# Yusheng-Xu/VGS-SVGS-Segmentation

Hardware: AMD Instinct MI355X
Metric: segmented points/sec (end-to-end VGS) (higher is better)
Workload: dtype f32

## Files before the change

### vgs-svgs-segmentation_amd/csrc/brick_table.hpp

```cpp
#ifndef BRICK_TABLE_HPP_
#define BRICK_TABLE_HPP_

#include "vgs_context.hpp"

struct Brick { unsigned long long key; unsigned long long occ; unsigned long long used; uint32_t first; uint32_t pad; };

__device__ __forceinline__ uint32_t hash_slot(uint64_t key, uint32_t hbits) {
  const uint32_t bx = (uint32_t)key & 0x1fffffu, by = (uint32_t)(key >> 21) & 0x1fffffu, bz = (uint32_t)(key >> 42);
  uint32_t h = bx * 0x9E3779B1u + by * 0x85EBCA77u + bz * 0xC2B2AE3Du;
  h ^= h >> 15;
  return (h * 0x2C1B3C6Du) >> (32 - hbits);
}

__device__ __forceinline__ unsigned long long brick_key(uint32_t nx, uint32_t ny, uint32_t nz) {
  return (((unsigned long long)(nz >> 2) << 42) | ((unsigned long long)(ny >> 2) << 21) | (unsigned long long)(nx >> 2)) + 1ull;
}
__device__ __forceinline__ int brick_local(uint32_t nx, uint32_t ny, uint32_t nz) {
  return (int)((nz & 1u) | ((ny & 1u) << 1) | ((nx & 1u) << 2) | ((nz & 2u) << 2) | ((ny & 2u) << 3) | ((nx & 2u) << 4));
}

static __global__ void k_brick_insert(const uint64_t* __restrict__ vox_code, const NodeRec* __restrict__ node, int64_t V,
                               Brick* __restrict__ table, uint32_t hbits) {
  const int64_t v = (int64_t)blockIdx.x * blockDim.x + threadIdx.x;
  const int lane = threadIdx.x & 63;
  unsigned long long key = 0ull, occ = 0ull, usd = 0ull;
  uint32_t first = 0xffffffffu;
  if (v < V) {
    const uint64_t code = vox_code[v];
    key = brick_key(vm_compact21(code >> 2), vm_compact21(code >> 1), vm_compact21(code));
    occ = 1ull << (code & 63ull);
    if (node && (node[v].flags & VGS_F_EIG)) usd = occ;
    first = (uint32_t)v;
  }
  for (int o = 1; o < 64; o <<= 1) {
    const unsigned long long ko = __shfl_up(key, o, 64), oo = __shfl_up(occ, o, 64), uo = __shfl_up(usd, o, 64);
    const uint32_t fo = (uint32_t)__shfl_up((int)first, o, 64);
    if (lane >= o && ko == key) { occ |= oo; usd |= uo; first = fo < first ? fo : first; }
  }
  const unsigned long long knext = __shfl_down(key, 1, 64);
  if (key == 0ull || (lane < 63 && knext == key)) return;
  const uint32_t mask = (1u << hbits) - 1u;
  uint32_t s = hash_slot(key, hbits);
  while (true) {
    const unsigned long long prev = atomicCAS(&table[s].key, 0ull, key);
    if (prev == 0ull || prev == key) break;
    s = (s + 1) & mask;
  }
  atomicOr(&table[s].occ, occ);
  if (usd) atomicOr(&table[s].used, usd);
  atomicMin(&table[s].first, first);
}

__device__ __forceinline__ int brick_find(const Brick* __restrict__ table, uint32_t hbits, uint32_t nx, uint32_t ny, uint32_t nz, bool* is_used) {
  const unsigned long long key = brick_key(nx, ny, nz);
  const uint32_t mask = (1u << hbits) - 1u;
  uint32_t s = hash_slot(key, hbits);
  while (true) {
    const unsigned long long k = table[s].key;
    if (k == key) break;
    if (k == 0ull) return -1;
    s = (s + 1) & mask;
  }
  const unsigned long long occ = table[s].occ;
  const int local = brick_local(nx, ny, nz);
  if (!((occ >> local) & 1ull)) return -1;
  *is_used = ((table[s].used >> local) & 1ull) != 0;
  const unsigned long long above = (local == 63) ? 0ull : (occ >> (local + 1));
  return (int)(table[s].first + (uint32_t)__popcll(above));
}


static __global__ void k_brick_clear(Brick* __restrict__ table, size_t H) {
  const size_t e = (size_t)blockIdx.x * blockDim.x + threadIdx.x;
  if (e >= H) return;
  ulonglong2* p = (ulonglong2*)&table[e];
  p[0] = make_ulonglong2(0ull, 0ull);
  p[1] = make_ulonglong2(0ull, 0x00000000ffffffffull);
}

static inline vgs_status vgs_build_bricks(vgs_ctx* c, const NodeRec* node) {
  const int64_t V = c->V;
  uint32_t hbits = 4;
  while ((1ull << hbits) < (uint64_t)(V + 16)) ++hbits;
  c->hbits = hbits;
  const size_t H = (size_t)1 << hbits;
  VGS_HIP_TRY(c, c->hkey.ensure(H * (sizeof(Brick) / 8)));
  hipLaunchKernelGGL(k_brick_clear, dim3((unsigned)((H + 255) / 256)), dim3(256), 0, c->stream, (Brick*)c->hkey.p, H);
  hipLaunchKernelGGL(k_brick_insert, dim3((unsigned)((V + 255) / 256)), dim3(256), 0, c->stream, c->vox_code.p, node, V, (Brick*)c->hkey.p, hbits);
  return VGS_OK;
}

#endif
```

### vgs-svgs-segmentation_amd/csrc/capi.hip

```cpp
#include <algorithm>
#include <cstdio>
#include <cstdlib>
#include <cstring>
#include <fstream>
#include <string>
#include <vector>

#include <dlfcn.h>

#include "vgs_context.hpp"

static thread_local std::string g_create_err;

static const char* const VGS_STAGE_NAMES[VGS_T_COUNT] = {"vgs:voxelize", "vgs:features", "vgs:adjacency", "vgs:localcut", "vgs:merge", "vgs:labels",
                                                         "vgs:total", "vgs:localcut_kernel", "vgs:supervoxels", "vgs:localcut_bulk", "", ""};
struct RoctxApi {
  int (*push)(const char*) = nullptr;
  int (*pop)() = nullptr;
  RoctxApi() {
    for (const char* name : {"librocprofiler-sdk-roctx.so.1", "librocprofiler-sdk-roctx.so", "libroctx64.so.4", "libroctx64.so"}) {
      void* h = dlopen(name, RTLD_LAZY | RTLD_LOCAL);
      if (!h) continue;
      push = (int (*)(const char*))dlsym(h, "roctxRangePushA");
      pop = (int (*)())dlsym(h, "roctxRangePop");
      if (push && pop) return;
      push = nullptr; pop = nullptr;
    }
  }
};
static const RoctxApi& roctx_api() { static const RoctxApi api; return api; }
struct RoctxRange {
  bool on;
  explicit RoctxRange(const char* name) : on(roctx_api().push != nullptr) { if (on) roctx_api().push(name); }
  ~RoctxRange() { if (on) roctx_api().pop(); }
};

template <typename F>
static vgs_status timed(vgs_ctx* c, int slot, F&& f, bool wait = true) {
  RoctxRange range(VGS_STAGE_NAMES[slot]);
  VGS_HIP_TRY(c, hipSetDevice(c->device));
  VGS_HIP_TRY(c, hipEventRecord(c->tev[slot][0], c->stream));
  c->tev_pending[slot] = false;
  vgs_status s = f();
  if (s != VGS_OK) return s;
  VGS_HIP_TRY(c, hipEventRecord(c->tev[slot][1], c->stream));
  c->tev_pending[slot] = true;
  if (wait) VGS_HIP_TRY(c, hipEventSynchronize(c->tev[slot][1]));
  return VGS_OK;
}

static vgs_status vgs_resolve_times(vgs_ctx* c) {
  for (int slot = 0; slot < VGS_T_COUNT; ++slot) {
    if (!c->tev_pending[slot]) continue;
    c->tev_pending[slot] = false;
    VGS_HIP_TRY(c, hipEventSynchronize(c->tev[slot][1]));
    float ms = 0.f;
    VGS_HIP_TRY(c, hipEventElapsedTime(&ms, c->tev[slot][0], c->tev[slot][1]));
    c->times[slot] = ms;
  }
  return VGS_OK;
}

void vgs_read_env_knobs(vgs_ctx* c) {
  VgsKnobs& k = c->K;
  auto geti = [](const char* n, int d) { const char* v = getenv(n); return v ? atoi(v) : d; };
  auto getf = [](const char* n, float d) { const char* v = getenv(n); return v ? (float)atof(v) : d; };
  auto has = [](const char* n) { return getenv(n) != nullptr; };
  k.a1_max = geti("VGS_A1MAX", k.a1_max); k.shell0 = getf("VGS_SHELL0", k.shell0); k.cap_frac = getf("VGS_CAPFRAC", k.cap_frac);
  k.dbg_stop = geti("VGS_DBG_STOP", k.dbg_stop); k.max_rounds = geti("VGS_ROUNDS", k.max_rounds); k.dbg_max_m = geti("VGS_DBG_MAXM", k.dbg_max_m); k.dbg_xl_from = geti("VGS_DBG_XL_FROM", k.dbg_xl_from);
  k.near_min_own = geti("VGS_NEARMINOWN", k.near_min_own); k.fv_blocks = geti("VGS_FV_BLOCKS", k.fv_blocks); k.only_class = geti("VGS_ONLY_CLASS", k.only_class);
  k.no_dense = has("VGS_NO_DENSE"); k.no_overlap = has("VGS_NO_OVERLAP"); k.no_near = has("VGS_NO_NEAR"); k.no_adjmasks = has("VGS_NO_ADJMASKS"); k.no_connbits = has("VGS_NO_CONNBITS"); k.no_pg_xl = has("VGS_NO_PG_XL"); k.no_sort32 = has("VGS_NO_SORT32"); k.no_pairlists = has("VGS_NO_PAIRLISTS"); k.no_vote = has("VGS_NO_VOTE"); k.vote_force = geti("VGS_VOTE_FORCE", 0); k.cross_lds_kb = geti("VGS_CROSS_LDS", k.cross_lds_kb); { int vp = geti("VGS_VOTE_PERIOD", k.vote_period); if (vp >= 2 && vp <= 4096 && (vp & (vp - 1)) == 0) k.vote_period = vp; } k.pg_wide = geti("VGS_PG_WIDE", k.pg_wide); k.pg_wide_frac = geti("VGS_PG_WIDEFRAC", k.pg_wide_frac); k.pg_min_frac = geti("VGS_PG_MINFRAC", k.pg_min_frac); k.ho_grid = geti("VGS_HO_GRID", k.ho_grid);
  k.debug = has("VGS_DEBUG");
}

static void vgs_charge_localcut_tail(vgs_ctx* c) {
  (void)vgs_resolve_times(c);
  const double t = (double)c->lc_tail.tail_ms;
  if (t > 0.0 && t < c->times[VGS_T_MERGE]) { c->times[VGS_T_LOCALCUT] += t; c->times[VGS_T_MERGE] -= t; }
  c->lc_tail.tail_ms = 0.f;
}

extern "C" {

vgs_status vgs_params_default_vgs(vgs_params* p) {
  if (!p) return VGS_E_ARG;
  std::memset(p, 0, sizeof(*p));
  p->method = 2;
  p->voxel_size = 0.15f; p->graph_size = 0.5f;
  p->sig_p = p->sig_n = p->sig_o = p->sig_e = p->sig_c = 0.2f;
  p->sig_w = 2.0f; p->cut_thred = 0.3f;
  p->points_min = 10; p->adjacency_min = 3; p->voxels_min = 3;
  p->seed_size = 0.25f; p->color_impt = 0.0f; p->spatial_impt = 0.25f; p->normal_impt = 0.75f;
  p->q7_count_as_index = 1;
  p->device = 0;
  return VGS_OK;
}

vgs_status vgs_params_default_svgs(vgs_params* p) {
  vgs_status s = vgs_params_default_vgs(p);
  if (s != VGS_OK) return s;
  p->method = 3;
  p->voxel_size = 0.05f; p->seed_size = 0.25f; p->graph_size = 0.5f;
  p->sig_w = 1.0f; p->cut_thred = 0.5f;
  p->vccs_mode = 1;
  return VGS_OK;
}

vgs_status vgs_parse_task_file(const char* path, vgs_params* p, char* in_name, char* out_name, int name_cap) {
  if (!path || !p) return VGS_E_ARG;
  std::ifstream f(path);
  if (!f.is_open()) return VGS_E_IO;
  std::vector<std::string> v;
  std::string line;
  while (std::getline(f, line)) {
    while (!line.empty() && (line.back() == '\r' || line.back() == '\n')) line.pop_back();
    v.push_back(line);
  }
  auto num = [&](size_t k) -> double { return k < v.size() ? std::atof(v[k].c_str()) : 0.0; };
  auto inum = [&](size_t k) -> int { return k < v.size() ? std::atoi(v[k].c_str()) : 0; };
  if (v.size() < 51) return VGS_E_IO;
  const int method = inum(24);
  if (method == 3) {
    if (v.size() < 61) return VGS_E_IO;
    vgs_params_default_svgs(p);
    p->voxel_size = (float)num(28); p->seed_size = (float)num(30); p->graph_size = (float)num(32);
    p->sig_p = (float)num(34); p->sig_n = (float)num(36); p->sig_o = (float)num(38); p->sig_e = (float)num(40);
    p->sig_c = (float)num(42); p->sig_w = (float)num(44);
    p->color_impt = (float)num(46); p->spatial_impt = (float)num(48); p->normal_impt = (float)num(50);
    p->cut_thred = (float)num(52);
    p->points_min = (int)num(54); p->voxels_min = inum(58); p->adjacency_min = inum(60);
  } else {
    vgs_params_default_vgs(p);
    p->voxel_size = (float)num(28); p->graph_size = (float)num(30);
    p->sig_p = (float)num(32); p->sig_n = (float)num(34); p->sig_o = (float)num(36); p->sig_e = (float)num(38);
    p->sig_c = (float)num(40); p->sig_w = (float)num(42); p->cut_thred = (float)num(44);
    p->points_min = inum(46); p->adjacency_min = inum(48); p->voxels_min = inum(50);
    p->method = 2;
  }
  if (in_name && name_cap > 0) { std::strncpy(in_name, v[15].c_str(), name_cap - 1); in_name[name_cap - 1] = 0; }
  if (out_name && name_cap > 0) { std::strncpy(out_name, v[21].c_str(), name_cap - 1); out_name[name_cap - 1] = 0; }
  return VGS_OK;
}

vgs_status vgs_create(const vgs_params* p, vgs_ctx** out) {
  if (!p || !out) return VGS_E_ARG;
  *out = nullptr;
  if (!(p->voxel_size > 0.f) || !(p->graph_size > 0.f) || !(p->sig_w != 0.f) || (p->method != 2 && p->method != 3)) {
    g_create_err = "vgs_create: voxel_size, graph_size must be > 0, sig_w != 0, method 2 or 3";
    return VGS_E_ARG;
  }
  if (p->vccs_mode != 0 && p->vccs_mode != 1) { g_create_err = "vgs_create: vccs_mode must be 0 (synchronous variant) or 1 (PCL's order)"; return VGS_E_ARG; }
  int ndev = 0;
  hipError_t e = hipGetDeviceCount(&ndev);
  if (e != hipSuccess || ndev <= 0) {
    g_create_err = std::string("vgs_create: no HIP device (") + hipGetErrorString(e) + "); this engine has no CPU path";
    return VGS_E_HIP;
  }
  if (p->device < 0 || p->device >= ndev) { g_create_err = "vgs_create: bad device ordinal"; return VGS_E_ARG; }
  vgs_ctx* c = new (std::nothrow) vgs_ctx();
  if (!c) return VGS_E_NOMEM;
  c->P = *p;
  c->device = p->device;
  int prio_lo = 0, prio_hi = 0;
  if (hipSetDevice(c->device) != hipSuccess || hipStreamCreateWithFlags(&c->stream, hipStreamNonBlocking) != hipSuccess ||
      hipDeviceGetStreamPriorityRange(&prio_lo, &prio_hi) != hipSuccess ||
      hipStreamCreateWithPriority(&c->stream2, hipStreamNonBlocking, prio_hi) != hipSuccess ||
      hipStreamCreateWithPriority(&c->stream3, hipStreamNonBlocking, prio_hi) != hipSuccess ||
      hipStreamCreateWithPriority(&c->stream4, hipStreamNonBlocking, prio_hi) != hipSuccess) {
    g_create_err = "vgs_create: hipSetDevice/hipStreamCreate failed";
    vgs_destroy(c);
    return VGS_E_HIP;
  }
  if (hipHostMalloc(&c->pin, 4096, hipHostMallocDefault) != hipSuccess) c->pin = nullptr;
  bool ok = hipStreamCreateWithFlags(&c->s_h2d, hipStreamNonBlocking) == hipSuccess &&
            hipStreamCreateWithFlags(&c->s_d2h, hipStreamNonBlocking) == hipSuccess &&
            hipEventCreateWithFlags(&c->ev_h2d, hipEventDisableTiming) == hipSuccess &&
            hipEventCreateWithFlags(&c->ev_d2h, hipEventDisableTiming) == hipSuccess &&
            hipEventCreateWithFlags(&c->ev_rb, hipEventDisableTiming) == hipSuccess &&
            hipEventCreateWithFlags(&c->ev_ho, hipEventDisableTiming) == hipSuccess &&
            hipEventCreateWithFlags(&c->ev_ho2, hipEventDisableTiming) == hipSuccess &&
            hipEventCreateWithFlags(&c->ev_fork, hipEventDisableTiming) == hipSuccess &&
            hipEventCreateWithFlags(&c->ev_join, hipEventDisableTiming) == hipSuccess;
  for (int i = 0; ok && i < 16; ++i) ok = hipEventCreate(&c->ev[i]) == hipSuccess;
  for (int i = 0; ok && i < VGS_T_COUNT; ++i) ok = hipEventCreate(&c->tev[i][0]) == hipSuccess && hipEventCreate(&c->tev[i][1]) == hipSuccess;
  if (!ok) { g_create_err = "vgs_create: hipStreamCreate/hipEventCreate failed"; vgs_destroy(c); return VGS_E_HIP; }
  vgs_read_env_knobs(c);
  *out = c;
  return VGS_OK;
}

void vgs_destroy(vgs_ctx* c) {
  if (!c) return;
  (void)hipSetDevice(c->device);
  if (c->stream) (void)hipStreamSynchronize(c->stream);
  if (c->stream2) (void)hipStreamSynchronize(c->stream2);
  if (c->stream3) (void)hipStreamSynchronize(c->stream3);
  if (c->stream4) (void)hipStreamSynchronize(c->stream4);
  if (c->s_h2d) (void)hipStreamSynchronize(c->s_h2d);
  if (c->s_d2h) (void)hipStreamSynchronize(c->s_d2h);
  c->xyz_buf[0].release(); c->xyz_buf[1].release(); c->pt_label_alt.release(); c->grow_state.release();
  c->code_a.release(); c->code_b.release(); c->perm_a.release(); c->perm_b.release(); c->sort_tmp.release();
  c->head_flag.release(); c->pt_vox.release(); c->vox_tile.release(); c->vox_code.release(); c->vox_start.release();
  c->xs.release(); c->ys.release(); c->zs.release();
  c->node.release(); c->used_ids.release(); c->used_rank.release();
  c->hkey.release(); c->hval.release(); c->offsets.release(); c->adj_masks.release(); c->adj_gtab.release(); c->adj_nvals.release(); c->adj_nrank.release(); c->adj_key.release(); c->adj_off.release(); c->adj_cnt.release(); c->adj_mused.release();
  c->nl_cnt.release(); c->nl_tot.release(); c->nl_ent.release(); c->lc_ctab.release(); c->pl_state.release(); c->pl_ent.release(); c->pl_work.release();
  c->sd_key.release(); c->sd_ids.release(); c->sd_vp.release(); c->sd_seg.release(); c->sd_tmp.release(); c->sd_part.release();
  c->sd_npts.release(); c->sd_nnodes.release(); c->sd_bbox.release(); c->sd_eig8.release(); c->sd_cen.release(); c->sd_cov.release(); c->sd_eval.release(); c->sd_evec.release();
  c->sd_apos.release(); c->sd_mom.release();
  c->sf_in.release(); c->sf_min.release(); c->sf_max.release(); c->sf_cls.release(); c->sf_maj.release(); c->sf_part.release(); c->sf_anchor.release(); c->sf_idx.release();
  c->sf_mean.release(); c->sf_var.release(); c->sf_nvalid.release(); c->sf_hist.release();
  c->sb_part.release(); c->sbt_in.release(); c->sbt_frame.release(); c->sbt_out.release(); c->sbt_idx.release();
  for (int f = 0; f < 2; ++f) { c->sb_frame[f].release(); c->sb_lo[f].release(); c->sb_hi[f].release(); c->sb_half[f].release(); c->sb_center[f].release(); }
  c->sg_lab.release(); c->sg_nrec.release(); c->sg_ridx.release(); c->sg_ework.release(); c->sg_meta.release(); c->sg_roff.release(); c->sg_rkey.release(); c->sg_rec.release(); c->sg_part.release(); c->sg_tmp.release();
  c->sg_ab.release(); c->sg_nodes.release(); c->sg_npairs.release(); c->sg_nfin.release(); c->sg_wsum.release(); c->sg_wmin.release(); c->sg_wmax.release();
  c->cmp_ref.release(); c->cmp_cell_i32.release(); c->cmp_ref_i32.release(); c->cmp_seg_i32.release(); c->cmp_cell_n.release(); c->cmp_ref_i64.release(); c->cmp_seg_i64.release();
  c->cmp_ref_iou.release(); c->cmp_seg_iou.release(); c->cmp_key.release(); c->cmp_meta.release(); c->cmp_work.release(); c->cmp_cstart.release(); c->cmp_rowstart.release();
  c->cmp_rsort.release(); c->cmp_rstart.release(); c->cmp_tmp.release();
  c->rf_label.release(); c->rf_batches.release(); c->rf_start.release(); c->rf_ids.release(); c->rf_cnt.release(); c->rf_nall.release();
  c->rf_rows.release(); c->rf_counts.release();
  c->ps_in.release(); c->ps_nnodes.release(); c->ps_key.release(); c->ps_val.release(); c->ps_seg.release(); c->ps_nn.release(); c->ps_tmp.release();
  c->ps_meta.release(); c->ps_part.release(); c->ps_d.release(); c->ps_f.release(); c->ps_npts.release();
  c->cl_off.release(); c->cl_idx.release(); c->conn.release(); c->evals.release(); c->lc_pending.release(); c->lc_defer.release(); c->lc_defer_flag.release(); c->csize.release(); c->attach.release(); c->cc_flags.release(); c->parent.release(); c->csz.release();
  c->vc_cen.release(); c->vc_nrm.release(); c->vc_dist.release(); c->vc_state.release(); c->vc_tile_start.release(); c->vc_cell.release(); c->vc_plive.release(); c->vc_tile_of.release(); c->vc_tchg.release(); c->vc_nbr_tiles.release(); c->vc_halo.release(); c->vc_tile_meta.release(); c->vc_pool.release(); c->vc_ring.release(); c->vc_dbg.release(); c->vc_label.release();
  c->vc_seedkey.release(); c->vc_sums.release(); c->vc_count.release(); c->vc_accu.release(); c->vc_alive.release();
  c->sv_label.release(); c->sv_key_a.release(); c->sv_key_b.release(); c->cell_code_a.release(); c->cell_code_b.release();
  c->cell_id_a.release(); c->cell_id_b.release(); c->cell_start.release();
  c->owned.release(); c->straddle.release(); c->mixsrc.release(); c->bnd_code.release(); c->bnd_root.release(); c->root_label.release();
  c->bnd_code2.release(); c->bnd_root2.release(); c->bnd_cnt.release(); c->broot.release();
  c->kept_rank.release(); c->vox_label.release(); c->pt_label.release(); c->counters.release(); c->work_ids.release();
  if (c->pin) (void)hipHostFree(c->pin);
  for (int i = 0; i < 16; ++i) if (c->ev[i]) (void)hipEventDestroy(c->ev[i]);
  for (int i = 0; i < VGS_T_COUNT; ++i) for (int k = 0; k < 2; ++k) if (c->tev[i][k]) (void)hipEventDestroy(c->tev[i][k]);
  if (c->stream) (void)hipStreamDestroy(c->stream);
  if (c->stream2) (void)hipStreamDestroy(c->stream2);
  if (c->stream3) (void)hipStreamDestroy(c->stream3);
  if (c->stream4) (void)hipStreamDestroy(c->stream4);
  if (c->s_h2d) (void)hipStreamDestroy(c->s_h2d);
  if (c->s_d2h) (void)hipStreamDestroy(c->s_d2h);
  if (c->ev_h2d) (void)hipEventDestroy(c->ev_h2d);
  if (c->ev_rb) (void)hipEventDestroy(c->ev_rb);
  if (c->ev_ho) (void)hipEventDestroy(c->ev_ho);
  if (c->ev_ho2) (void)hipEventDestroy(c->ev_ho2);
  if (c->ev_fork) (void)hipEventDestroy(c->ev_fork);
  if (c->ev_join) (void)hipEventDestroy(c->ev_join);
  if (c->ev_d2h) (void)hipEventDestroy(c->ev_d2h);
  delete c;
}

vgs_status vgs_set_params(vgs_ctx* c, const vgs_params* p) {
  if (!c || !p) return VGS_E_ARG;
  if (!(p->voxel_size > 0.f) || !(p->graph_size > 0.f) || !(p->sig_w != 0.f)) { c->err = "vgs_set_params: voxel_size, graph_size > 0, sig_w != 0"; return VGS_E_ARG; }
  if (p->method != c->P.method || p->device != c->P.device) { c->err = "vgs_set_params: method and device are fixed at vgs_create"; return VGS_E_ARG; }
  if (p->vccs_mode != 0 && p->vccs_mode != 1) { c->err = "vgs_set_params: vccs_mode must be 0 (synchronous variant) or 1 (PCL's order)"; return VGS_E_ARG; }
  int keep = ST_SEGMENTED;
  const vgs_params& o = c->P;
  if (p->cut_thred != o.cut_thred || p->sig_p != o.sig_p || p->sig_n != o.sig_n || p->sig_o != o.sig_o || p->sig_e != o.sig_e ||
      p->sig_c != o.sig_c || p->sig_w != o.sig_w || p->adjacency_min != o.adjacency_min || p->voxels_min != o.voxels_min ||
      p->q7_count_as_index != o.q7_count_as_index)
    keep = ST_ADJACENCY;
  if (p->graph_size != o.graph_size) keep = ST_FEATURES;
  if (p->points_min != o.points_min) keep = ST_VOXELS;
  if (p->voxel_size != o.voxel_size || p->seed_size != o.seed_size || p->color_impt != o.color_impt ||
      p->spatial_impt != o.spatial_impt || p->normal_impt != o.normal_impt || p->vccs_mode != o.vccs_mode)
    keep = ST_POINTS;
  if (c->stage > keep) c->stage = keep;
  if (keep < ST_SEGMENTED) { c->sd_valid = false; c->sb_valid[0] = c->sb_valid[1] = false; c->sg_valid = false; c->cmp_valid = false; c->rf_valid = false; c->cmp_own_cells = -1; c->sg_halo_valid = false; c->sg_own_K = -1; c->rf_halo_valid = false; c->rf_band_n = -1; }
  if (keep == ST_POINTS && c->P.method == 3 && !c->sv_labels_external) { c->sv_have_labels = false; c->sv_max_label = 0; c->sv_label_n = -1; }
  c->P = *p;
  return VGS_OK;
}

const char* vgs_last_error_string(const vgs_ctx* c) { return c ? c->err.c_str() : g_create_err.c_str(); }

static vgs_status set_points_common(vgs_ctx* c, int64_t n, int32_t stride_bytes) {
  if (n < 0 || (stride_bytes != 12 && stride_bytes != 16)) { c->err = "set_points: n >= 0 and stride_bytes 12 or 16 required"; return VGS_E_ARG; }
  if (n >= (int64_t)1 << 31) { c->err = "set_points: more than 2^31-1 points"; return VGS_E_UNSUPPORTED; }
  c->N = n;
  c->stride_f = stride_bytes / 4;
  c->stage = ST_POINTS;
  c->sd_valid = false;
  c->sb_valid[0] = c->sb_valid[1] = false;
  c->sg_valid = false; c->cmp_valid = false; c->rf_valid = false; c->cmp_own_cells = -1; c->sg_halo_valid = false; c->sg_own_K = -1; c->rf_halo_valid = false; c->rf_band_n = -1;
  c->grid_covers = false;
  c->counts[VGS_N_POINTS] = n;
  for (int i = 0; i < VGS_T_COUNT; ++i) { c->times[i] = 0; c->tev_pending[i] = false; }
  c->sv_have_labels = false; c->sv_labels_external = false; c->sv_max_label = 0; c->sv_label_n = -1;
  c->n_own = -1; c->own_first = 0;
  return VGS_OK;
}

vgs_status vgs_set_points(vgs_ctx* c, const float* xyz_host, int64_t n, int32_t stride_bytes) {
  if (!c || (!xyz_host && n > 0)) return VGS_E_ARG;
  VGS_HIP_TRY(c, hipSetDevice(c->device));
  vgs_status s = set_points_common(c, n, stride_bytes);
  if (s != VGS_OK) return s;
  DevBuf<float>& buf = c->xyz_buf[c->xyz_cur];
  VGS_HIP_TRY(c, buf.ensure((size_t)n * c->stride_f + 4));
  if (n > 0) VGS_HIP_TRY(c, hipMemcpyAsync(buf.p, xyz_host, (size_t)n * stride_bytes, hipMemcpyHostToDevice, c->stream));
  VGS_HIP_TRY(c, hipStreamSynchronize(c->stream));
  c->xyz = buf.p;
  return VGS_OK;
}

vgs_status vgs_stage_points(vgs_ctx* c, const float* xyz_host, int64_t n, int32_t stride_bytes) {
  if (!c || (!xyz_host && n > 0)) return VGS_E_ARG;
  if (n < 0 || (stride_bytes != 12 && stride_bytes != 16)) { c->err = "vgs_stage_points: n >= 0 and stride_bytes 12 or 16 required"; return VGS_E_ARG; }
  if (n >= (int64_t)1 << 31) { c->err = "vgs_stage_points: more than 2^31-1 points"; return VGS_E_UNSUPPORTED; }
  VGS_HIP_TRY(c, hipSetDevice(c->device));
  if (c->staged) VGS_HIP_TRY(c, hipEventSynchronize(c->ev_h2d));
  DevBuf<float>& buf = c->xyz_buf[1 - c->xyz_cur];
  VGS_HIP_TRY(c, buf.ensure((size_t)n * (stride_bytes / 4) + 4));
  if (n > 0) VGS_HIP_TRY(c, hipMemcpyAsync(buf.p, xyz_host, (size_t)n * stride_bytes, hipMemcpyHostToDevice, c->s_h2d));
  VGS_HIP_TRY(c, hipEventRecord(c->ev_h2d, c->s_h2d));
  c->staged = true; c->staged_n = n; c->staged_stride = stride_bytes;
  return VGS_OK;
}

vgs_status vgs_commit_points(vgs_ctx* c) {
  if (!c) return VGS_E_ARG;
  if (!c->staged) { c->err = "vgs_commit_points: no staged cloud (vgs_stage_points first)"; return VGS_E_STATE; }
  VGS_HIP_TRY(c, hipSetDevice(c->device));
  VGS_HIP_TRY(c, hipStreamWaitEvent(c->stream, c->ev_h2d, 0));
  vgs_status s = set_points_common(c, c->staged_n, c->staged_stride);
  if (s != VGS_OK) return s;
  c->xyz_cur = 1 - c->xyz_cur;
  c->xyz = c->xyz_buf[c->xyz_cur].p;
  c->staged = false;
  return VGS_OK;
}

vgs_status vgs_host_alloc(void** p, uint64_t bytes) {
  if (!p) return VGS_E_ARG;
  *p = nullptr;
  return hipHostMalloc(p, bytes > 0 ? (size_t)bytes : 1, hipHostMallocDefault) == hipSuccess ? VGS_OK : VGS_E_NOMEM;
}
vgs_status vgs_host_free(void* p) { return (!p || hipHostFree(p) == hipSuccess) ? VGS_OK : VGS_E_HIP; }
vgs_status vgs_host_register(void* p, uint64_t bytes) {
  if (!p || bytes == 0) return VGS_E_ARG;
  return hipHostRegister(p, (size_t)bytes, hipHostRegisterDefault) == hipSuccess ? VGS_OK : VGS_E_HIP;
}
vgs_status vgs_host_unregister(void* p) { return (p && hipHostUnregister(p) == hipSuccess) ? VGS_OK : VGS_E_HIP; }

vgs_status vgs_set_points_device(vgs_ctx* c, const float* xyz_dev, int64_t n, int32_t stride_bytes) {
  if (!c || (!xyz_dev && n > 0)) return VGS_E_ARG;
  VGS_HIP_TRY(c, hipSetDevice(c->device));
  vgs_status s = set_points_common(c, n, stride_bytes);
  if (s != VGS_OK) return s;
  c->xyz = xyz_dev;
  return VGS_OK;
}

}

static vgs_status do_voxelize(vgs_ctx* c, bool wait) {
  if (!c) return VGS_E_ARG;
  if (c->stage < ST_POINTS) { c->err = "vgs_voxelize: no input cloud (setInputCloud/getCloudPointNum first)"; return VGS_E_STATE; }
  vgs_status s = timed(c, VGS_T_VOXELIZE, [&] { return vgs_stage_voxelize(c); }, wait);
  if (s == VGS_OK) c->stage = ST_VOXELS;
  return s;
// ... 111 lines not shown
    for (uint32_t x : cnt) e += x;
    c->counts[VGS_N_ADJ] = e;
  }
  if (c->stage >= ST_SEGMENTED && c->U > 0 && c->counts[VGS_N_PAIRS] < 0) {
    std::vector<uint32_t> ev((size_t)c->U);
    VGS_HIP_TRY(c, hipMemcpy(ev.data(), c->evals.p, ev.size() * 4, hipMemcpyDeviceToHost));
    int64_t tot = 0;
    for (uint32_t x : ev) tot += x;
    c->counts[VGS_N_PAIRS] = tot;
  }
  for (int i = 0; i < VGS_N_COUNTS; ++i) counts[i] = c->counts[i];
  return VGS_OK;
}

vgs_status vgs_get_stage_times(vgs_ctx* c, double* ms) {
  if (!c || !ms) return VGS_E_ARG;
  { vgs_status sr = vgs_resolve_times(c); if (sr != VGS_OK) return sr; }
  if (c->P.method == 2 && c->stage >= ST_SEGMENTED)
    c->times[VGS_T_TOTAL] = c->times[VGS_T_VOXELIZE] + c->times[VGS_T_FEATURES] + c->times[VGS_T_ADJACENCY] + c->times[VGS_T_LOCALCUT] + c->times[VGS_T_MERGE];
  for (int i = 0; i < VGS_T_COUNT; ++i) ms[i] = c->times[i];
  return VGS_OK;
}

vgs_status vgs_get_schedule_counters(vgs_ctx* c, int64_t* out) { return vgs_get_schedule_counters_ex(c, out, 8); }

vgs_status vgs_get_schedule_counters_ex(vgs_ctx* c, int64_t* out, int32_t n) {
  if (!c || !out || n < 0 || n > 16) return VGS_E_ARG;
  for (int i = 0; i < n; ++i) out[i] = c->lc_diag[i];
  return VGS_OK;
}

vgs_status vgs_get_bbox(vgs_ctx* c, double* b) {
  if (!c || !b) return VGS_E_ARG;
  if (c->stage < ST_VOXELS) { c->err = "vgs_get_bbox: voxelize first"; return VGS_E_STATE; }
  for (int a = 0; a < 3; ++a) { b[a] = c->box.min[a]; b[3 + a] = c->box.max[a]; }
  return VGS_OK;
}

vgs_status vgs_get_voxel_table(vgs_ctx* c, uint32_t* key, int32_t* start, int32_t* point_idx) {
  if (!c) return VGS_E_ARG;
  if (c->stage < ST_VOXELS) { c->err = "vgs_get_voxel_table: voxelize first"; return VGS_E_STATE; }
  VGS_HIP_TRY(c, hipSetDevice(c->device));
  if (key && c->V > 0) {
    std::vector<uint64_t> code((size_t)c->V);
    VGS_HIP_TRY(c, hipMemcpy(code.data(), c->vox_code.p, code.size() * 8, hipMemcpyDeviceToHost));
    for (int64_t v = 0; v < c->V; ++v) {
      key[3 * v + 0] = vm_compact21(code[v] >> 2);
      key[3 * v + 1] = vm_compact21(code[v] >> 1);
      key[3 * v + 2] = vm_compact21(code[v]);
    }
  }
  if (start) {
    if (c->V > 0) VGS_HIP_TRY(c, hipMemcpy(start, c->vox_start.p, (size_t)(c->V + 1) * 4, hipMemcpyDeviceToHost));
    else start[0] = 0;
  }
  if (point_idx && c->Nf > 0) VGS_HIP_TRY(c, hipMemcpy(point_idx, c->perm_b.p, (size_t)c->Nf * 4, hipMemcpyDeviceToHost));
  return VGS_OK;
}

vgs_status vgs_get_voxel_centers(vgs_ctx* c, float* center) {
  if (!c || !center) return VGS_E_ARG;
  if (c->stage < ST_VOXELS) { c->err = "vgs_get_voxel_centers: voxelize first"; return VGS_E_STATE; }
  if (c->V == 0) return VGS_OK;
  std::vector<uint64_t> code((size_t)c->V);
  VGS_HIP_TRY(c, hipMemcpy(code.data(), c->vox_code.p, code.size() * 8, hipMemcpyDeviceToHost));
  const float res_f = c->P.voxel_size;
  const float mn[3] = {(float)c->box.min[0], (float)c->box.min[1], (float)c->box.min[2]};
  for (int64_t v = 0; v < c->V; ++v) {
    center[3 * v + 0] = vm_voxel_center(vm_compact21(code[v] >> 2), res_f, mn[0]);
    center[3 * v + 1] = vm_voxel_center(vm_compact21(code[v] >> 1), res_f, mn[1]);
    center[3 * v + 2] = vm_voxel_center(vm_compact21(code[v]), res_f, mn[2]);
  }
  return VGS_OK;
}

vgs_status vgs_get_point_voxel(vgs_ctx* c, int32_t* out) {
  if (!c || !out) return VGS_E_ARG;
  if (c->stage < ST_VOXELS) { c->err = "vgs_get_point_voxel: voxelize first"; return VGS_E_STATE; }
  if (c->N == 0) return VGS_OK;
  if (c->Nf == 0) {
    for (int64_t j = 0; j < c->N; ++j) out[j] = -1;
    return VGS_OK;
  }
  std::vector<uint32_t> perm((size_t)c->N), pv((size_t)c->N);
  VGS_HIP_TRY(c, hipMemcpy(perm.data(), c->perm_b.p, perm.size() * 4, hipMemcpyDeviceToHost));
  VGS_HIP_TRY(c, hipMemcpy(pv.data(), c->pt_vox.p, pv.size() * 4, hipMemcpyDeviceToHost));
  for (int64_t j = 0; j < c->N; ++j) out[perm[j]] = (pv[j] == 0xffffffffu) ? -1 : (int32_t)pv[j];
  return VGS_OK;
}

vgs_status vgs_get_attributes(vgs_ctx* c, float* centroid, float* normal, float* eigen8, uint8_t* used) {
  if (!c) return VGS_E_ARG;
  if (c->stage < ST_FEATURES) { c->err = "vgs_get_attributes: features first"; return VGS_E_STATE; }
  if (c->V == 0) return VGS_OK;
  std::vector<NodeRec> nd((size_t)c->V);
  VGS_HIP_TRY(c, hipMemcpy(nd.data(), c->node.p, nd.size() * sizeof(NodeRec), hipMemcpyDeviceToHost));
  for (int64_t v = 0; v < c->V; ++v) {
    for (int a = 0; a < 3; ++a) {
      if (centroid) centroid[3 * v + a] = nd[v].c[a];
      if (normal) normal[3 * v + a] = nd[v].n[a];
    }
    if (eigen8) for (int a = 0; a < 8; ++a) eigen8[8 * v + a] = nd[v].f[a];
    if (used) used[v] = (nd[v].flags & VGS_F_EIG) ? 1 : 0;
  }
  return VGS_OK;
}

}

static vgs_status vgs_build_lists(vgs_ctx* c, int32_t which, std::vector<std::vector<int32_t>>& L, bool ordered = false) {
  const int64_t V = c->V, U = c->U;
  if (which == 0 && c->P.method == 2 && V > 0) {
    VGS_HIP_TRY(c, hipSetDevice(c->device));
    L.assign((size_t)V, {});
    const int64_t chunk = std::min<int64_t>(V, 65536);
    DevBuf<uint64_t> fk; DevBuf<uint32_t> fc, fn, fid;
    VGS_HIP_TRY(c, fk.ensure((size_t)chunk * c->adj_stride)); VGS_HIP_TRY(c, fc.ensure(chunk)); VGS_HIP_TRY(c, fn.ensure(chunk)); VGS_HIP_TRY(c, fid.ensure(chunk));
    std::vector<uint32_t> ids((size_t)chunk), cnt((size_t)chunk);
    std::vector<uint64_t> keys((size_t)chunk * c->adj_stride);
    vgs_status st = VGS_OK;
    for (int64_t v0 = 0; v0 < V && st == VGS_OK; v0 += chunk) {
      const int64_t m = std::min(chunk, V - v0);
      for (int64_t k = 0; k < m; ++k) ids[(size_t)k] = (uint32_t)(v0 + k);
      if (hipMemcpy(fid.p, ids.data(), (size_t)m * 4, hipMemcpyHostToDevice) != hipSuccess) { st = VGS_E_HIP; break; }
      st = vgs_run_adjacency(c, true, fk.p, fc.p, fn.p, c->adj_r2, fid.p, m);
      if (st == VGS_OK && hipStreamSynchronize(c->stream) != hipSuccess) st = VGS_E_HIP;
      if (st == VGS_OK && (hipMemcpy(cnt.data(), fc.p, (size_t)m * 4, hipMemcpyDeviceToHost) != hipSuccess ||
                           hipMemcpy(keys.data(), fk.p, (size_t)m * c->adj_stride * 8, hipMemcpyDeviceToHost) != hipSuccess)) st = VGS_E_HIP;
      if (st != VGS_OK) break;
      for (int64_t k = 0; k < m; ++k) {
        std::vector<int32_t>& l = L[(size_t)(v0 + k)];
        l.resize(cnt[(size_t)k]);
        for (uint32_t q = 0; q < cnt[(size_t)k]; ++q) l[q] = (int32_t)(uint32_t)keys[(size_t)k * c->adj_stride + q];
      }
    }
    fk.release(); fc.release(); fn.release(); fid.release();
    if (st == VGS_E_HIP) c->err = "vgs_get_lists: full adjacency pass failed";
    return st;
  }
  std::vector<uint32_t> used_ids((size_t)U), cnt((size_t)U);
  std::vector<uint64_t> keys;
  std::vector<uint8_t> flag;
  std::vector<int32_t> attach;
  if (ordered && which >= 1 && U > 0) {
    VGS_HIP_TRY(c, hipSetDevice(c->device));
    VGS_HIP_TRY(c, hipMemcpy(used_ids.data(), c->used_ids.p, (size_t)U * 4, hipMemcpyDeviceToHost));
    std::vector<uint16_t> ord;
    std::vector<uint32_t> kk, lcnt;
    std::vector<int32_t> lids;
    const uint8_t* lflag = which == 1 ? (const uint8_t*)nullptr : c->conn.p + (size_t)U * c->adj_stride;
    vgs_status so = vgs_cut_order(c, ord, kk, true, lflag, &lcnt, &lids);
    if (so != VGS_OK) return so;
    L.assign((size_t)V, {});
    size_t at = 0;
    for (int64_t u = 0; u < U; ++u) {
      L[used_ids[(size_t)u]].assign(lids.begin() + (ptrdiff_t)at, lids.begin() + (ptrdiff_t)(at + lcnt[(size_t)u]));
      at += lcnt[(size_t)u];
    }
    if (which == 3) {
      attach.resize((size_t)V);
      VGS_HIP_TRY(c, hipMemcpy(attach.data(), c->attach.p, (size_t)V * 4, hipMemcpyDeviceToHost));
      for (int64_t i = 0; i < V; ++i)
        if (attach[i] >= 0) { L[i].push_back(attach[i]); L[attach[i]].push_back((int32_t)i); }
    }
    return VGS_OK;
  }
  if (U > 0) {
    VGS_HIP_TRY(c, hipSetDevice(c->device));
    VGS_HIP_TRY(c, hipMemcpy(used_ids.data(), c->used_ids.p, (size_t)U * 4, hipMemcpyDeviceToHost));
    keys.resize((size_t)U * c->adj_stride);
// ... 176 lines not shown
```

### vgs-svgs-segmentation_amd/csrc/clusters.hip

```cpp
#include <cstring>
#include <string.h>

#include <rocprim/rocprim.hpp>

#include "vgs_context.hpp"

__global__ void k_cluster_keys(const uint32_t* __restrict__ pt_vox, const int32_t* __restrict__ vox_label, int64_t nf, uint32_t K,
                               uint32_t* __restrict__ key) {
  const int64_t j = (int64_t)blockIdx.x * blockDim.x + threadIdx.x;
  if (j >= nf) return;
  const uint32_t v = pt_vox[j];
  const int32_t l = v == 0xffffffffu ? -1 : vox_label[v];
  key[j] = l < 0 ? K : (uint32_t)l;
}
__global__ void k_cluster_offsets(const uint32_t* __restrict__ key, int64_t nf, uint32_t K, int64_t* __restrict__ off) {
  const uint32_t k = blockIdx.x * blockDim.x + threadIdx.x;
  if (k > K) return;
  int64_t lo = 0, hi = nf;
  while (lo < hi) { const int64_t mid = (lo + hi) >> 1; if (key[mid] < k) lo = mid + 1; else hi = mid; }
  off[k] = lo;
}

vgs_status vgs_clusters_on_device(vgs_ctx* c) {
  if (c->cl_valid) return VGS_OK;
  const int64_t K = c->counts[VGS_N_KEPT], nf = c->Nf;
  VGS_HIP_TRY(c, hipSetDevice(c->device));
  VGS_HIP_TRY(c, c->cl_off.ensure((size_t)K + 2));
  VGS_HIP_TRY(c, c->cl_idx.ensure((size_t)(nf > 0 ? nf : 1)));
  if (nf == 0 || K == 0) {
    VGS_HIP_TRY(c, hipMemsetAsync(c->cl_off.p, 0, ((size_t)K + 1) * sizeof(int64_t), c->stream));
    VGS_HIP_TRY(c, hipStreamSynchronize(c->stream));
    c->cl_valid = true;
    return VGS_OK;
  }
  VGS_HIP_TRY(c, c->code_a.ensure((size_t)nf)); VGS_HIP_TRY(c, c->code_b.ensure((size_t)nf));
  uint32_t* key_in = (uint32_t*)c->code_a.p;
  uint32_t* key_out = key_in + nf;
  uint32_t* val_out = (uint32_t*)c->cl_idx.p;
  const int TB = 256;
  const unsigned nb = (unsigned)((nf + TB - 1) / TB);
  hipLaunchKernelGGL(k_cluster_keys, dim3(nb), dim3(TB), 0, c->stream, c->pt_vox.p, c->vox_label.p, nf, (uint32_t)K, key_in);
  unsigned bits = 1;
  while (bits < 32 && (1ull << bits) <= (unsigned long long)K) ++bits;
  size_t tmp = 0;
  VGS_HIP_TRY(c, rocprim::radix_sort_pairs(nullptr, tmp, key_in, key_out, c->perm_b.p, val_out, (size_t)nf, 0, bits, c->stream));
  VGS_HIP_TRY(c, c->sort_tmp.ensure(tmp));
  VGS_HIP_TRY(c, rocprim::radix_sort_pairs(c->sort_tmp.p, tmp, key_in, key_out, c->perm_b.p, val_out, (size_t)nf, 0, bits, c->stream));
  hipLaunchKernelGGL(k_cluster_offsets, dim3((unsigned)((K + 1 + TB - 1) / TB)), dim3(TB), 0, c->stream, key_out, nf, (uint32_t)K, c->cl_off.p);
  VGS_HIP_TRY(c, hipGetLastError());
  VGS_HIP_TRY(c, hipStreamSynchronize(c->stream));
  c->cl_valid = true;
  return VGS_OK;
}

extern "C" vgs_status vgs_get_clusters_device(vgs_ctx* c, const int64_t** offsets_dev, const int32_t** point_idx_dev) {
  if (!c || !offsets_dev || !point_idx_dev) return VGS_E_ARG;
  if (c->stage < ST_SEGMENTED) { c->err = "vgs_get_clusters_device: segment first (drawColorMapofPointsinClusters precedes getClusterIdx, VS:1006)"; return VGS_E_STATE; }
  vgs_status s = vgs_clusters_on_device(c);
  if (s != VGS_OK) return s;
  *offsets_dev = c->cl_off.p;
  *point_idx_dev = c->cl_idx.p;
  return VGS_OK;
}
```

### vgs-svgs-segmentation_amd/csrc/localcut.hip

```cpp
#include <algorithm>
#include <cmath>
#include <cstring>
#include <vector>
#include <cstdio>
#include <cstdlib>

#include "vgs_context.hpp"

#ifndef LC_TB
#define LC_TB 256
#endif
#ifndef LC_SMALL_CAP
#define LC_SMALL_CAP 4096
#endif
#define LC_NBIN 2048

#define LC_TBINS 64
struct LcParams {
  VgsWeightParams W;
  float cut;
  int prune_unused;
  float d2_stop;
  float ctab_scale;
  const float* ctab;
// ... 830 lines not shown
    uint32_t* const wbits = c->cb_enabled ? c->conn_bits.p : (uint32_t*)nullptr;
    uint32_t* const ids_xl_pg = c->work_ids.p + (10 + LW_HO_BINS) * U;
    unsigned int* const d_nxl = (unsigned int*)(c->counters.p + 56);
    const bool pg_xl = c->cb_R <= 10 && !c->K.no_pg_xl && n_above_d != 0u;
    c->lc_tail.pg_xl_queued = pg_xl && nabc[3] > 0;
    VGS_HIP_TRY(c, hipEventRecord(c->ev_ho2, c->stream2));
    VGS_HIP_TRY(c, hipStreamWaitEvent(c->stream4, c->ev_ho2, 0));
    if (nabc[3] > 0)
      hipLaunchKernelGGL((k_localcut_pg<PG_D>), dim3(vgs_xcd_grid(nabc[3])), dim3(512), 0, c->stream2, ids_d, 0, 1, (const unsigned int*)nullptr, nabc[3], 1, c->adj_key.p,
                         c->adj_cnt.p, c->adj_stride, c->adj_off.p, c->node.p, LP, PLw, G, c->conn.p, cnt, ids_g, d_ng, c->evals.p, c->lc_pending.p, wbits, c->cb_R,
                         c->cb_words, LcGate{nullptr, 0u}, pg_xl ? ids_xl_pg : (uint32_t*)nullptr, pg_xl ? d_nxl : (unsigned int*)nullptr);
    if (nabc[3] > 0 && pg_xl)
      hipLaunchKernelGGL((k_localcut_pg<PG_XL>), dim3(256), dim3(64 * PG_XL_NW), 0, c->stream2, ids_xl_pg, 0, 1, d_nxl, 0u, 0, c->adj_key.p,
                         c->adj_cnt.p, c->adj_stride, c->adj_off.p, c->node.p, LP, PLw, G, c->conn.p, cnt, ids_g, d_ng, c->evals.p, c->lc_pending.p, wbits, c->cb_R,
                         c->cb_words, LcGate{nullptr, 0u}, (uint32_t*)nullptr, (unsigned int*)nullptr);
    if (nabc[2] > 0)
      hipLaunchKernelGGL((k_localcut_pg<PG_C>), dim3(vgs_xcd_grid(nabc[2])), dim3(256), 0, c->stream2, ids_c, 0, 1, (const unsigned int*)nullptr, nabc[2], 1, c->adj_key.p,
                         c->adj_cnt.p, c->adj_stride, c->adj_off.p, c->node.p, LP, PLw, G, c->conn.p, cnt, ids_g, d_ng, c->evals.p, c->lc_pending.p, wbits, c->cb_R,
                         c->cb_words, LcGate{nullptr, 0u}, (uint32_t*)nullptr, (unsigned int*)nullptr);
    if (nabc[5] > 0)
      hipLaunchKernelGGL((k_localcut_pg<PG_C0>), dim3(vgs_xcd_grid(nabc[5])), dim3(256), 0, c->stream4, ids_c0, 0, 1, (const unsigned int*)nullptr, nabc[5], 1, c->adj_key.p,
                         c->adj_cnt.p, c->adj_stride, c->adj_off.p, c->node.p, LP, PLw, G, c->conn.p, cnt, ids_g, d_ng, c->evals.p, c->lc_pending.p, wbits, c->cb_R,
                         c->cb_words, LcGate{nullptr, 0u}, (uint32_t*)nullptr, (unsigned int*)nullptr);
    VGS_HIP_TRY(c, hipEventRecord(c->ev[12], c->stream4));
    VGS_HIP_TRY(c, hipEventRecord(c->ev[5], c->stream2));
    VGS_HIP_TRY(c, hipStreamWaitEvent(c->stream2, c->ev[12], 0));
    hipLaunchKernelGGL((k_localcut_dense<DN_LARGE>), dim3(n_wide < 4 * GRID_G ? n_wide : 4 * GRID_G), dim3(512), 0, c->stream2, ids_g, 0, 1, d_ng, c->adj_key.p,
                       c->adj_cnt.p, c->adj_stride, c->node.p, LP, c->conn.p, cnt, ids_g2, d_ng2, c->evals.p, LcGate{nullptr, 0u}, (uint32_t*)nullptr, (unsigned int*)nullptr);
  } else {
    if (nabc[3] + nabc[5] > 0) {
      VGS_HIP_TRY(c, hipStreamWaitEvent(c->stream4, c->ev[2], 0));
      if (nabc[5] > 0)
        hipLaunchKernelGGL((k_localcut_wave<WAVE_C0, LCAP_C0, NW_C>), dim3(((nabc[5] + 7) / 8) * 8), dim3(64 * NW_C), 0, c->stream4, (const uint32_t*)nullptr, 0,
                           ids_c0, (int)nabc[5], (const unsigned int*)nullptr, c->adj_key.p, c->adj_cnt.p, c->adj_stride, c->node.p, WP, c->conn.p, cnt,
                           ids_g, d_ng, c->evals.p, dbg_buf, c->adj_have_off ? c->adj_off.p : (const uint16_t*)nullptr);
      if (nabc[3] > 0)
      hipLaunchKernelGGL((k_localcut_wave<WAVE_D, LCAP_D, NW_D>), dim3(((nabc[3] + 7) / 8) * 8), dim3(64 * NW_D), 0, c->stream4, (const uint32_t*)nullptr, 0,
                         ids_d, (int)nabc[3], (const unsigned int*)nullptr, c->adj_key.p, c->adj_cnt.p, c->adj_stride, c->node.p, WP, c->conn.p, cnt,
                         ids_g, d_ng, c->evals.p, dbg_buf, c->adj_have_off ? c->adj_off.p : (const uint16_t*)nullptr);
      VGS_HIP_TRY(c, hipEventRecord(c->ev[12], c->stream4));
    }
    if (nabc[2] > 0)
      hipLaunchKernelGGL((k_localcut_wave<WAVE_C, LCAP_C, NW_C>), dim3(((nabc[2] + 7) / 8) * 8), dim3(64 * NW_C), 0, c->stream2, (const uint32_t*)nullptr, 0, ids_c, (int)nabc[2], (const unsigned int*)nullptr,
                         c->adj_key.p, c->adj_cnt.p, c->adj_stride, c->node.p, WP, c->conn.p, cnt, ids_g, d_ng, c->evals.p, dbg_buf, c->adj_have_off ? c->adj_off.p : (const uint16_t*)nullptr);
    VGS_HIP_TRY(c, hipEventRecord(c->ev[5], c->stream2));
    if (nabc[3] + nabc[5] > 0) VGS_HIP_TRY(c, hipStreamWaitEvent(c->stream2, c->ev[12], 0));
    vgs_status st = VGS_OK;
    const unsigned int ncd = nabc[2] + nabc[3] + nabc[5];
    if (ncd > 0) {
      if (!dense) st = launch_block(c->stream2, ids_g, ncd < GRID_G ? ncd : GRID_G, false, d_ng, 0);
      else
        hipLaunchKernelGGL((k_localcut_dense<DN_LARGE>), dim3(ncd < 4 * GRID_G ? ncd : 4 * GRID_G), dim3(512), 0, c->stream2, ids_g, 0, 1, d_ng, c->adj_key.p,
                           c->adj_cnt.p, c->adj_stride, c->node.p, LP, c->conn.p, cnt, ids_g2, d_ng2, c->evals.p, LcGate{nullptr, 0u}, (uint32_t*)nullptr, (unsigned int*)nullptr);
    }
    if (st != VGS_OK) return st;
  }
  VGS_HIP_TRY(c, hipEventRecord(c->ev[3], c->stream2));
  const bool sort32 = LW_SORT32 != 0 && !c->K.no_sort32 && vm_cut_threshold(1.0f, LP.cut, 1) >= 0.5f;
#define LW_LAUNCH_1W(MAXM_, LCAP_, SAMPLED_, GRID, STRM, ...)                                                                                        \
  do {                                                                                                                                             \
    if (sort32) hipLaunchKernelGGL((k_localcut_wave<MAXM_, LCAP_, 1, SAMPLED_, true>), GRID, dim3(64), 0, STRM, __VA_ARGS__);                        \
    else hipLaunchKernelGGL((k_localcut_wave<MAXM_, LCAP_, 1, SAMPLED_, false>), GRID, dim3(64), 0, STRM, __VA_ARGS__);                             \
  } while (0)
  if (nabc[6] > 0)
    LW_LAUNCH_1W(WAVE_B, LCAP_B, true, dim3(vgs_xcd_grid(nabc[6])), c->stream3, (const uint32_t*)nullptr, 0,
                       ids_s, (int)nabc[6], (const unsigned int*)nullptr, c->adj_key.p, c->adj_cnt.p, c->adj_stride, c->node.p, WP, c->conn.p, cnt, ids_f, d_nf, c->evals.p, dbg_buf, c->adj_have_off ? c->adj_off.p : (const uint16_t*)nullptr);
  if (nabc[1] > 0)
    LW_LAUNCH_1W(WAVE_B, LCAP_B, false, dim3(vgs_xcd_grid(nabc[1])), c->stream3, (const uint32_t*)nullptr, 0,
                       ids_b, (int)nabc[1], (const unsigned int*)nullptr, c->adj_key.p, c->adj_cnt.p, c->adj_stride, c->node.p, WP, c->conn.p, cnt, ids_f, d_nf, c->evals.p, dbg_buf, c->adj_have_off ? c->adj_off.p : (const uint16_t*)nullptr);
  VGS_HIP_TRY(c, hipEventRecord(c->ev[8], c->stream3));
  VGS_HIP_TRY(c, hipEventRecord(c->ev[10], c->stream));
  if (n_bulk > 0) {
    LwParams WPA = WP;
    unsigned int grid_a = vgs_xcd_grid(nabc[4]) + vgs_xcd_grid(nabc[0]);
    if (early_sizes) {
      WPA.n_first_dev = d_nabc + 4; WPA.n_main_dev = d_nabc + 0;
      grid_a = vgs_xcd_grid(n_bulk) + 8u;
    }
    LW_LAUNCH_1W(WAVE_A, LCAP_A, false, dim3(grid_a), c->stream, ids_a1, (int)nabc[4],
                       ids_a, (int)nabc[0], (const unsigned int*)nullptr, c->adj_key.p, c->adj_cnt.p, c->adj_stride, c->node.p, WPA, c->conn.p, cnt, ids_f, d_nf, c->evals.p, dbg_buf, c->adj_have_off ? c->adj_off.p : (const uint16_t*)nullptr);
#undef LW_LAUNCH_1W
  }
  VGS_HIP_TRY(c, hipEventRecord(c->ev[11], c->stream));
  const unsigned int nab = nabc[0] + nabc[1] + nabc[4] + nabc[6];
  unsigned int grid_f = std::min<unsigned int>(nab, std::min<unsigned int>(GRID_F, nab / 32 + 256));
  if (c->K.ho_grid != 0) {
    int n_cu = 256;
    (void)hipDeviceGetAttribute(&n_cu, hipDeviceAttributeMultiprocessorCount, c->device);
    const unsigned int fit = c->K.ho_grid > 0 ? (unsigned int)c->K.ho_grid : (unsigned int)n_cu * LD_SMALL_WG_PER_CU;
    grid_f = std::min(grid_f, fit);
  }
  {
    VGS_HIP_TRY(c, hipStreamWaitEvent(c->stream3, c->ev[11], 0));
    if (dense && nab > 0)
      hipLaunchKernelGGL(k_ho_lists, dim3((unsigned)((U + 1023) / 1024)), dim3(256), 0, c->stream3, c->lc_pending.p, U, ids_f, U, d_nf, cnt, d_gate,
                         (c->pl_enabled && c->K.pg_min_frac > 0) ? (unsigned int)(U / c->K.pg_min_frac) : 0xffffffffu);
    if (dense && nab > 0) VGS_HIP_TRY(c, hipEventRecord(c->ev_ho, c->stream3));
    vgs_status st = VGS_OK;
    if (!dense) {
      st = launch_block(c->stream3, ids_f, grid_f, true, d_nf, 0);
    } else if (grid_f > 0 && c->pl_enabled) {
      c->pl_enabled_at_launch = true;
      const LcGate g_few = {d_gate, LC_FEW}, g_many = {d_gate, LC_MANY};
      const uint32_t* ids4[LW_HO_BINS]; const unsigned int* nd4[LW_HO_BINS];
      for (int k = 0; k < LW_HO_BINS; ++k) { ids4[k] = ids_f + (size_t)k * U; nd4[k] = d_nf + k; }
      auto pair_lists = [&]() { return PairLists{(const uint2*)c->pl_state.p, c->pl_ent.p, c->pl_state.p + (size_t)c->V * 9, c->pl_w_ring}; };
      const PgGeom G = {c->vox_code.p, c->P.voxel_size, (float)c->box.min[0], (float)c->box.min[1], (float)c->box.min[2], c->adj_r2};
      {
      hipLaunchKernelGGL((k_localcut_dense<DN_SMALL>), dim3(grid_f), dim3(256), 0, c->stream3, ids_f, (int)U, LW_HO_BINS, d_nf, c->adj_key.p, c->adj_cnt.p,
                         c->adj_stride, c->node.p, LP, c->conn.p, cnt, ids_f2, d_nf2, c->evals.p, g_few, (uint32_t*)nullptr, (unsigned int*)nullptr);
      VGS_HIP_TRY(c, hipStreamWaitEvent(c->stream4, c->ev_ho, 0));
      st = vgs_pairlists_build(c, c->stream4, ids4, nd4, nullptr, LW_HO_BINS, true, LP.ctab, LP.ctab_scale, LP.d2_stop, 1, g_many, false);
      if (st == VGS_OK && c->pl_enabled) {
        hipLaunchKernelGGL((k_localcut_pg<PG_SMALL>), dim3(grid_f), dim3(256), 0, c->stream4, ids_f, (int)U, LW_HO_BINS, d_nf, 0u, 0, c->adj_key.p, c->adj_cnt.p,
                           c->adj_stride, c->adj_off.p, c->node.p, LP, pair_lists(), G, c->conn.p, cnt, ids_f2, d_nf2, c->evals.p, (uint8_t*)nullptr,
                           (uint32_t*)nullptr, 0, 0, g_many, (uint32_t*)nullptr, (unsigned int*)nullptr);
      } else if (st == VGS_OK) {
        hipLaunchKernelGGL((k_localcut_dense<DN_SMALL>), dim3(grid_f), dim3(256), 0, c->stream4, ids_f, (int)U, LW_HO_BINS, d_nf, c->adj_key.p, c->adj_cnt.p,
                           c->adj_stride, c->node.p, LP, c->conn.p, cnt, ids_f2, d_nf2, c->evals.p, g_many, (uint32_t*)nullptr, (unsigned int*)nullptr);
      }
      }
    } else if (grid_f > 0) {
      hipLaunchKernelGGL((k_localcut_dense<DN_SMALL>), dim3(grid_f), dim3(256), 0, c->stream3, ids_f, (int)U, LW_HO_BINS, d_nf, c->adj_key.p, c->adj_cnt.p,
                         c->adj_stride, c->node.p, LP, c->conn.p, cnt, ids_f2, d_nf2, c->evals.p, LcGate{nullptr, 0u}, (uint32_t*)nullptr, (unsigned int*)nullptr);
    }
    if (st != VGS_OK) return st;
    if (grid_f > 0 && dense && c->pl_enabled_at_launch) {
      VGS_HIP_TRY(c, hipEventRecord(c->ev_ho2, c->stream4));
      VGS_HIP_TRY(c, hipStreamWaitEvent(c->stream3, c->ev_ho2, 0));
    }
    VGS_HIP_TRY(c, hipEventRecord(c->ev[4], c->stream3));
  }
  VGS_HIP_TRY(c, hipStreamWaitEvent(c->stream, c->ev[8], 0));
  VGS_HIP_TRY(c, hipStreamWaitEvent(c->stream, c->ev[5], 0));
  if (nabc[3] + nabc[5] > 0) VGS_HIP_TRY(c, hipStreamWaitEvent(c->stream, c->ev[12], 0));
  if (c->K.no_overlap) {
    VGS_HIP_TRY(c, hipStreamWaitEvent(c->stream, c->ev[4], 0));
    VGS_HIP_TRY(c, hipStreamWaitEvent(c->stream, c->ev[3], 0));
    if (c->cb_enabled)
      hipLaunchKernelGGL(k_conn_bits, dim3((unsigned)U), dim3(64), 0, c->stream, c->lc_pending.p, U, c->adj_cnt.p, c->adj_stride, c->conn.p, c->adj_off.p,
                         c->cb_R, c->cb_words, c->conn_bits.p, CbLists{}, 0);
    VGS_HIP_TRY(c, hipMemsetAsync(c->lc_pending.p, 0, (size_t)U, c->stream));
  }
  if (c->pl_enabled_at_launch) c->lc_tail.gated = true;
  c->lc_tail.grid_f = grid_f;
  for (int k = 0; k < 5; ++k) c->lc_tail.nabc[k] = nabc[k];
  c->lc_tail.nabc[2] += nabc[5];
  VGS_HIP_TRY(c, hipEventRecord(c->ev[13], c->stream));
  c->counts[13] = nabc[0] + nabc[4]; c->counts[14] = nabc[1] + nabc[2] + nabc[5] + nabc[6]; c->counts[15] = nabc[3];
  c->counts[VGS_N_PAIRS] = -1;
  VGS_HIP_TRY(c, hipGetLastError());
  return VGS_OK;
}

vgs_status vgs_localcut_finish_queue(vgs_ctx* c, hipStream_t s) {
  if (!c->lc_tail.open || !c->pin || c->lc_tail.rb_queued) return VGS_OK;
  VGS_HIP_TRY(c, hipStreamWaitEvent(s, c->ev[4], 0));
  VGS_HIP_TRY(c, hipStreamWaitEvent(s, c->ev[3], 0));
  VGS_HIP_TRY(c, hipEventRecord(c->ev[7], s));
  VGS_HIP_TRY(c, hipMemcpyAsync(c->pin, c->counters.p, 64 * sizeof(unsigned long long), hipMemcpyDeviceToHost, s));
  c->lc_tail.rb_queued = true;
  return VGS_OK;
}

vgs_status vgs_localcut_finish(vgs_ctx* c, hipStream_t s, unsigned int* n_deferred) {
  if (n_deferred) *n_deferred = 0;
// ... 203 lines not shown
```

### vgs-svgs-segmentation_amd/csrc/merge.hip

```cpp
#include <cstring>
#include <string.h>
#include <utility>

#include <rocprim/rocprim.hpp>

#include "vgs_context.hpp"

struct MgParams {
  VgsWeightParams W;
  int adjacency_min;
  int q7;
  int64_t V;
};

#define MF_CAP_TRIPS 8
template <int W, int T>
__device__ __forceinline__ void mf_load(const uint8_t* __restrict__ flags, int limit, int k0, int sub, uint8_t (&f)[T]) {
#pragma unroll
  for (int q = 0; q < T; ++q) {
    const int k = k0 + q * W + sub;
    f[q] = flags[k < limit ? k : 0];
  }
}
template <int W, int T>
__device__ __forceinline__ void mf_append(const uint8_t (&f)[T], uint8_t* __restrict__ zero, int n, int k0, int sub,
                                          unsigned long long mine, uint16_t* list, int& cnt) {
#pragma unroll
  for (int q = 0; q < T; ++q) {
    const int k = k0 + q * W + sub;
    const bool in = k < n, set = in && f[q] != 0;
    const unsigned long long mk = __ballot(set) & mine;
    if (set) list[cnt + (int)__builtin_amdgcn_mbcnt_hi((unsigned)(mk >> 32), __builtin_amdgcn_mbcnt_lo((unsigned)mk, 0u))] = (uint16_t)k;
    else if (in && zero) zero[k] = 0;
    cnt += __popcll(mk);
  }
}
__device__ __forceinline__ void mf_wave_sync() {
  __builtin_amdgcn_fence(__ATOMIC_ACQ_REL, "workgroup");
  __builtin_amdgcn_wave_barrier();
}

#ifndef CX_ROWS
#define CX_ROWS 2
#endif
__global__ __launch_bounds__(64) __attribute__((amdgpu_waves_per_eu(8))) void k_cross(const uint32_t* __restrict__ used_ids, const uint32_t* __restrict__ used_rank, int64_t U,
                                              const uint64_t* __restrict__ adj_key, const uint32_t* __restrict__ adj_cnt,
                                              int adj_stride, const uint8_t* __restrict__ conn, uint8_t* __restrict__ mutual,
                                              uint32_t* __restrict__ csize, uint32_t* __restrict__ parent,
                                              const uint16_t* __restrict__ gtab, int gstride, const uint8_t* __restrict__ nrank, float inv_res2,
                                              const uint8_t* __restrict__ pending, uint32_t* __restrict__ defer_list,
                                              unsigned int* __restrict__ n_defer, const uint32_t* __restrict__ work, int n_work,
                                              const uint16_t* __restrict__ adj_off, int cb_R,
                                              const uint32_t* __restrict__ cbits, int cb_words, uint8_t* __restrict__ defer_flag, LcGate gate,
                                              const uint8_t* __restrict__ owned = nullptr) {
  if (!lc_gate_open_early(gate)) return;
  constexpr int W = 64 / CX_ROWS;
  const int lane = threadIdx.x, grp = lane / W, sub = lane % W;
  __shared__ uint32_t s_rank4[64];
  __shared__ uint16_t s_list[CX_ROWS][MF_CAP_TRIPS * W];
  constexpr int T = 4, CAP = MF_CAP_TRIPS * W;
  const uint32_t rank4 = gtab ? ((const uint32_t*)nrank)[lane] : 0u;
  int64_t u;
  bool live;
  if (work) {
    const int w = (int)blockIdx.x * CX_ROWS + grp;
    live = w < n_work;
    u = live ? (int64_t)work[w] : 0;
  } else {
    const int64_t ngroups = (U + CX_ROWS - 1) / CX_ROWS;
    const int64_t g = vgs_xcd_item(blockIdx.x, ngroups);
    u = g * CX_ROWS + grp;
    live = g < ngroups && u < U;
    if (!live) u = 0;
  }
  const uint64_t* row = adj_key + u * adj_stride;
  const uint8_t* crow = conn + u * adj_stride;
  uint8_t* mrow = mutual + u * adj_stride;
  const uint8_t put_off = pending ? pending[u] : (uint8_t)0;
  const uint32_t i = used_ids[u];
  const int n = (int)adj_cnt[u];
  uint8_t f[T];
  mf_load<W, T>(crow, adj_stride, 0, sub, f);
  if (gtab) s_rank4[lane] = rank4;
  __syncthreads();
  const uint8_t* s_rank = (const uint8_t*)s_rank4;
  if (!live) return;
  if (put_off) { if (sub == 0) { defer_list[atomicAdd(n_defer, 1u)] = (uint32_t)u; if (defer_flag) defer_flag[u] = 1; } return; }
  bool touches_pending = false;
  uint16_t* list = s_list[grp];
// ... 239 lines not shown
  while (true) {
    const uint32_t p = __hip_atomic_load(&parent[x], __ATOMIC_RELAXED, __HIP_MEMORY_SCOPE_AGENT);
    if (p == x) return x;
    x = p;
  }
}
__device__ __forceinline__ void k_flatten_body(uint32_t* __restrict__ parent, int64_t V, const uint8_t* __restrict__ owned, uint32_t* __restrict__ csz,
                                               uint32_t* s_root, unsigned int* s_cnt);
__global__ void k_flatten(uint32_t* __restrict__ parent, int64_t V, const uint8_t* __restrict__ owned, uint32_t* __restrict__ csz) {
  __shared__ uint32_t s_root[32];
  __shared__ unsigned int s_cnt[32];
  if (threadIdx.x < 32) { s_root[threadIdx.x] = 0xffffffffu; s_cnt[threadIdx.x] = 0u; }
  __syncthreads();
  k_flatten_body(parent, V, owned, csz, s_root, s_cnt);
  __syncthreads();
  if (threadIdx.x < 32 && s_cnt[threadIdx.x]) atomicAdd(&csz[s_root[threadIdx.x]], s_cnt[threadIdx.x]);
}
__device__ __forceinline__ void k_flatten_body(uint32_t* __restrict__ parent, int64_t V, const uint8_t* __restrict__ owned, uint32_t* __restrict__ csz,
                                               uint32_t* s_root, unsigned int* s_cnt) {
  int64_t v = (int64_t)blockIdx.x * blockDim.x + threadIdx.x;
  if (v >= V) return;
  const uint32_t r = uf_root(parent, (uint32_t)v);
  __hip_atomic_store(&parent[v], r, __ATOMIC_RELAXED, __HIP_MEMORY_SCOPE_AGENT);
  const bool counted = !owned || owned[v];
  const bool self = r == (uint32_t)v;
  if (counted && self) atomicAdd(&csz[r], 1u);
  unsigned long long todo = __ballot(counted && !self);
  if (!counted || self) return;
  const int lane = threadIdx.x & 63;
  while (todo) {
    const int l0 = __ffsll((long long)todo) - 1;
    const uint32_t r0 = (uint32_t)__shfl((int)r, l0, 64);
    const unsigned long long same = __ballot(r == r0) & todo;
    if (lane == l0) {
      const unsigned int n = (unsigned int)__popcll(same);
      unsigned int h = (r0 * 2654435761u) >> 27;
      bool put = false;
      for (int probe = 0; probe < 4 && !put; ++probe, h = (h + 1u) & 31u) {
        const uint32_t prev = atomicCAS(&s_root[h], 0xffffffffu, r0);
        if (prev == 0xffffffffu || prev == r0) { atomicAdd(&s_cnt[h], n); put = true; }
      }
      if (!put) atomicAdd(&csz[r0], n);
    }
    todo &= ~same;
    if ((same >> lane) & 1ull) break;
  }
}

__global__ __launch_bounds__(1024) void k_root_flags(const uint32_t* __restrict__ parent, const uint32_t* __restrict__ csz, int64_t V, int voxels_min,
                                                     uint32_t* __restrict__ keep_flag, unsigned int* __restrict__ n_roots) {
  __shared__ unsigned int s_cnt;
  if (threadIdx.x == 0) s_cnt = 0;
  __syncthreads();
  int64_t v = (int64_t)blockIdx.x * blockDim.x + threadIdx.x;
  bool root = false;
  if (v < V) {
    root = parent[v] == (uint32_t)v;
    keep_flag[v] = (root && (int)csz[v] > voxels_min) ? 1u : 0u;
  }
  const unsigned long long m = __ballot(root);
  if ((threadIdx.x & 63) == 0 && m) atomicAdd(&s_cnt, (unsigned int)__popcll(m));
  __syncthreads();
  if (threadIdx.x == 0 && s_cnt) atomicAdd(n_roots, s_cnt);
}

__global__ void k_voxel_labels(const uint32_t* __restrict__ parent, const uint32_t* __restrict__ keep_flag,
                               const uint32_t* __restrict__ keep_rank, int64_t V, int32_t* __restrict__ vox_label,
                               unsigned int* __restrict__ n_kept) {
  int64_t v = (int64_t)blockIdx.x * blockDim.x + threadIdx.x;
  if (v >= V) return;
  const uint32_t r = parent[v];
  vox_label[v] = keep_flag[r] ? (int32_t)keep_rank[r] : -1;
  if (v == V - 1) *n_kept = keep_rank[v] + keep_flag[v];
}

__global__ void k_point_labels(const uint32_t* __restrict__ perm, const uint32_t* __restrict__ pt_vox, const int32_t* __restrict__ vox_label,
                               int64_t N, int32_t* __restrict__ label) {
  int64_t j = (int64_t)blockIdx.x * blockDim.x + threadIdx.x;
  if (j >= N) return;
  const uint32_t v = pt_vox[j];
  label[perm[j]] = (v == 0xffffffffu) ? -1 : vox_label[v];
}

vgs_status vgs_ensure_point_labels(vgs_ctx* c) {
  if (!c->pt_labels_pending) return VGS_OK;
  c->pt_labels_pending = false;
  VGS_HIP_TRY(c, hipSetDevice(c->device));
  if (c->d2h_open && c->d2h_src == c->pt_label.p) { VGS_HIP_TRY(c, hipEventSynchronize(c->ev_d2h)); c->d2h_open = false; }
  const int TB = 256;
  hipLaunchKernelGGL(k_point_labels, dim3((unsigned)((c->N + TB - 1) / TB)), dim3(TB), 0, c->stream, c->perm_b.p, c->pt_vox.p, c->vox_label.p,
                     c->N, c->pt_label.p);
  VGS_HIP_TRY(c, hipEventRecord(c->ev[15], c->stream));
  c->labels_event_valid = true;
  VGS_HIP_TRY(c, hipStreamSynchronize(c->stream));
  return VGS_OK;
}

static VgsWeightParams make_weight_params_m(const vgs_params& p) {
  VgsWeightParams W;
  W.inv_sig_p = 1.0f / p.sig_p; W.inv_sig_n = 1.0f / p.sig_n; W.inv_sig_o = 1.0f / p.sig_o;
  W.inv_sig_e = 1.0f / p.sig_e; W.inv_sig_c = 1.0f / p.sig_c;
  W.inv_sig_w2 = 1.0f / (p.sig_w * p.sig_w);
  W.svgs = (p.method == 3) ? 1 : 0;
  return W;
}

__global__ void k_local_weights(const uint64_t* __restrict__ row, int n, const NodeRec* __restrict__ node, VgsWeightParams W,
                                int32_t* __restrict__ ids, float* __restrict__ out) {
  const int64_t t = (int64_t)blockIdx.x * blockDim.x + threadIdx.x;
  if (t < n) ids[t] = (int32_t)(uint32_t)row[t];
  if (t >= (int64_t)n * n) return;
  const int a = (int)(t / n), b = (int)(t % n);
  out[t] = vm_pair_weight(node[(uint32_t)row[a]], node[(uint32_t)row[b]], W);
}

extern "C" vgs_status vgs_get_local_weights(vgs_ctx* c, int32_t node_id, int32_t* n_out, int32_t* ids, float* weights) {
  if (!c || !n_out) return VGS_E_ARG;
  if (c->stage < ST_ADJACENCY) { c->err = "vgs_get_local_weights: adjacency first"; return VGS_E_STATE; }
  if (node_id < 0 || node_id >= c->V) { c->err = "vgs_get_local_weights: node id out of range"; return VGS_E_ARG; }
  VGS_HIP_TRY(c, hipSetDevice(c->device));
  uint32_t u = 0xffffffffu;
  VGS_HIP_TRY(c, hipMemcpy(&u, c->used_rank.p + node_id, 4, hipMemcpyDeviceToHost));
  if (u == 0xffffffffu) { *n_out = 0; return VGS_OK; }
  uint32_t n = 0;
  VGS_HIP_TRY(c, hipMemcpy(&n, c->adj_cnt.p + u, 4, hipMemcpyDeviceToHost));
  *n_out = (int32_t)n;
  if (!ids || !weights || n == 0) return VGS_OK;
  DevBuf<float> d_w; DevBuf<int32_t> d_ids;
  VGS_HIP_TRY(c, d_w.ensure((size_t)n * n)); VGS_HIP_TRY(c, d_ids.ensure(n));
  const int64_t total = (int64_t)n * n;
  hipLaunchKernelGGL(k_local_weights, dim3((unsigned)((total + 255) / 256)), dim3(256), 0, c->stream, c->adj_key.p + (size_t)u * c->adj_stride, (int)n,
                     c->node.p, make_weight_params_m(c->P), d_ids.p, d_w.p);
  hipError_t e = hipStreamSynchronize(c->stream);
  if (e == hipSuccess) e = hipMemcpy(weights, d_w.p, (size_t)total * 4, hipMemcpyDeviceToHost);
  if (e == hipSuccess) e = hipMemcpy(ids, d_ids.p, (size_t)n * 4, hipMemcpyDeviceToHost);
  d_w.release(); d_ids.release();
  if (e != hipSuccess) { c->err = std::string("vgs_get_local_weights: ") + hipGetErrorString(e); return VGS_E_HIP; }
  return VGS_OK;
}

vgs_status vgs_stage_merge(vgs_ctx* c) {
  c->cl_valid = false;
  c->sd_valid = false;
  c->sb_valid[0] = c->sb_valid[1] = false;
  c->sg_valid = false; c->cmp_valid = false; c->rf_valid = false; c->cmp_own_cells = -1; c->sg_halo_valid = false; c->sg_own_K = -1; c->rf_halo_valid = false; c->rf_band_n = -1;
  const int64_t V = c->V, U = c->U, N = c->N;
  c->bnd_unique = -1;
  c->counts[VGS_N_CLUSTERS] = 0; c->counts[VGS_N_KEPT] = 0; c->counts[VGS_N_ISOLATED] = 0; c->counts[VGS_N_REATTACHED] = 0;
  if (c->d2h_open && c->d2h_src == c->pt_label.p) std::swap(c->pt_label, c->pt_label_alt);
  VGS_HIP_TRY(c, c->pt_label.ensure(N > 0 ? N : 1));
  if (V == 0) {
    if (N > 0) {
      VGS_HIP_TRY(c, hipMemsetAsync(c->pt_label.p, 0xff, N * sizeof(int32_t), c->stream));
      VGS_HIP_TRY(c, hipEventRecord(c->ev[15], c->stream));
      c->labels_event_valid = true;
    }
    c->pt_labels_pending = false;
    return VGS_OK;
  }
  MgParams MP;
  MP.W = make_weight_params_m(c->P);
  MP.adjacency_min = c->P.adjacency_min;
  MP.q7 = c->P.q7_count_as_index;
  MP.V = V;
  const int TB = 256;
  const unsigned nbV = (unsigned)((V + TB - 1) / TB);
  VGS_HIP_TRY(c, c->csize.ensure(V)); VGS_HIP_TRY(c, c->attach.ensure(V)); VGS_HIP_TRY(c, c->cc_flags.ensure(V));
  VGS_HIP_TRY(c, c->parent.ensure(V)); VGS_HIP_TRY(c, c->csz.ensure(V)); VGS_HIP_TRY(c, c->kept_rank.ensure(V + 1));
  VGS_HIP_TRY(c, c->vox_label.ensure(V));
  VGS_HIP_TRY(c, c->counters.ensure(64));
  uint64_t* mcnt = c->counters.p + 48;
  VGS_HIP_TRY(c, hipMemsetAsync(mcnt, 0, 8 * sizeof(uint64_t), c->stream));
  hipLaunchKernelGGL(k_merge_init, dim3(nbV), dim3(TB), 0, c->stream, c->parent.p, c->csize.p, c->attach.p, c->cc_flags.p, c->csz.p, V);
  uint8_t* mutual = nullptr;
  unsigned int n_cand = 0, n_succ = 0;
  bool compressed = false, united = false;
  if (U > 0) {
    if (c->conn.cap < 2 * (size_t)U * c->adj_stride) { c->err = "connect buffer missing (local cut stage not run)"; return VGS_E_STATE; }
    mutual = c->conn.p + (size_t)U * c->adj_stride;
    const uint16_t* gt = (c->P.method == 2 && c->adj_have_gtab) ? c->adj_gtab.p : nullptr;
    const float inv_res2 = 1.0f / (c->P.voxel_size * c->P.voxel_size);
    if (c->have_region) { vgs_status so = vgs_compute_owned(c); if (so != VGS_OK) return so; }
    const uint8_t* owned_early = c->have_region ? c->owned.p : (const uint8_t*)nullptr;
    unsigned int* d_ndefer = (unsigned int*)(c->counters.p + 13);
    const bool early_union = c->lc_tail.open && !c->K.no_overlap;
    if (early_union) VGS_HIP_TRY(c, c->lc_defer_flag.ensure((size_t)U));
    const bool use_bits = c->cb_enabled && c->P.method == 2 && c->adj_have_off;
    const uint16_t* cb_off = use_bits ? c->adj_off.p : (const uint16_t*)nullptr;
    const int cb_lut = c->cb_R;
    const uint32_t* cb_bits = use_bits ? c->conn_bits.p : (const uint32_t*)nullptr;
    const LcGate g_first = {(c->lc_tail.open && c->lc_tail.gated) ? (const unsigned int*)(c->counters.p + 57) : (const unsigned int*)nullptr, LC_FEW};
    const size_t first_lds = (c->lc_tail.open && c->K.cross_lds_kb > 0) ? (size_t)c->K.cross_lds_kb * 1024 : 0;
    hipLaunchKernelGGL(k_cross, dim3(vgs_xcd_grid((U + CX_ROWS - 1) / CX_ROWS)), dim3(64), first_lds, c->stream, c->used_ids.p, c->used_rank.p, U, c->adj_key.p, c->adj_cnt.p,
                       c->adj_stride, c->conn.p, mutual, c->csize.p, c->parent.p, gt, c->adj_gstride, c->adj_nrank.p, inv_res2,
                       c->lc_tail.open ? c->lc_pending.p : (const uint8_t*)nullptr, c->lc_defer.p, d_ndefer, (const uint32_t*)nullptr, 0,
                       cb_off, cb_lut, cb_bits, c->cb_words, early_union ? c->lc_defer_flag.p : (uint8_t*)nullptr, g_first, owned_early);
    hipStream_t s = c->stream;
    if (early_union) {
      VGS_HIP_TRY(c, hipEventRecord(c->ev_fork, c->stream));
      VGS_HIP_TRY(c, hipStreamWaitEvent(c->stream3, c->ev_fork, 0));
      s = c->stream3;
      { vgs_status sq = vgs_localcut_finish_queue(c, s); if (sq != VGS_OK) return sq; }
      hipLaunchKernelGGL(k_compress, dim3(nbV), dim3(TB), 0, c->stream, c->parent.p, V);
      hipLaunchKernelGGL(k_union_mutual, dim3((unsigned)((U + UM_ROWS - 1) / UM_ROWS)), dim3(64), first_lds, c->stream, c->used_ids.p, U, c->adj_key.p, c->adj_cnt.p,
                         c->adj_stride, mutual, c->attach.p, owned_early, c->parent.p, 0, c->lc_defer_flag.p, (const uint32_t*)nullptr, 0, g_first);
      compressed = true; united = true;
    }
    unsigned int n_defer = 0;
    {
      vgs_status sf = vgs_localcut_finish(c, s, &n_defer);
      if (sf != VGS_OK) return sf;
    }
    if (c->lc_tail.many) {
      if (s != c->stream) {
        VGS_HIP_TRY(c, hipEventRecord(c->ev_join, s));
        VGS_HIP_TRY(c, hipStreamWaitEvent(c->stream, c->ev_join, 0));
        s = c->stream;
      }
      hipLaunchKernelGGL(k_merge_init, dim3(nbV), dim3(TB), 0, c->stream, c->parent.p, c->csize.p, c->attach.p, c->cc_flags.p, c->csz.p, V);
      hipLaunchKernelGGL(k_cross, dim3(vgs_xcd_grid((U + CX_ROWS - 1) / CX_ROWS)), dim3(64), 0, c->stream, c->used_ids.p, c->used_rank.p, U, c->adj_key.p, c->adj_cnt.p,
                         c->adj_stride, c->conn.p, mutual, c->csize.p, c->parent.p, gt, c->adj_gstride, c->adj_nrank.p, inv_res2,
                         (const uint8_t*)nullptr, c->lc_defer.p, d_ndefer, (const uint32_t*)nullptr, 0, cb_off, cb_lut, cb_bits, c->cb_words, (uint8_t*)nullptr,
                         LcGate{nullptr, 0u}, owned_early);
      compressed = false; united = false;
      n_defer = 0;
    }
    if (n_defer > 0) {
      hipLaunchKernelGGL(k_cross, dim3((n_defer + CX_ROWS - 1) / CX_ROWS), dim3(64), 0, s, c->used_ids.p, c->used_rank.p, U, c->adj_key.p, c->adj_cnt.p,
                         c->adj_stride, c->conn.p, mutual, c->csize.p, early_union ? (uint32_t*)nullptr : c->parent.p, gt, c->adj_gstride, c->adj_nrank.p, inv_res2,
                         (const uint8_t*)nullptr, c->lc_defer.p, d_ndefer, c->lc_defer.p, (int)n_defer, cb_off, cb_lut, cb_bits, c->cb_words, (uint8_t*)nullptr, LcGate{nullptr, 0u});
      if (s != c->stream) {
        VGS_HIP_TRY(c, hipEventRecord(c->ev_fork, s));
        VGS_HIP_TRY(c, hipStreamWaitEvent(c->stream, c->ev_fork, 0));
      }
      if (early_union)
        hipLaunchKernelGGL(k_union_mutual, dim3((n_defer + UM_ROWS - 1) / UM_ROWS), dim3(64), 0, c->stream, c->used_ids.p, U, c->adj_key.p, c->adj_cnt.p,
                           c->adj_stride, mutual, c->attach.p, owned_early, c->parent.p, 0, (const uint8_t*)nullptr, c->lc_defer.p, (int)n_defer, LcGate{nullptr, 0u});
    }
    VGS_HIP_TRY(c, c->work_ids.ensure((size_t)U + 16));
    unsigned int* d_ncand = (unsigned int*)(mcnt + 0);
    unsigned int* d_changed = (unsigned int*)(mcnt + 1);
    hipLaunchKernelGGL(k_cc_candidates, dim3((unsigned)((U + TB - 1) / TB)), dim3(TB), 0, s, c->used_ids.p, U, c->adj_mused.p,
                       c->csize.p, MP.adjacency_min, c->cc_flags.p, c->work_ids.p, d_ncand);
    const bool hide = !c->have_region && vgs_can_split_readback(c) && !early_union;
    if (hide) {
      vgs_status sb = vgs_readback_begin(c, d_ncand, 4);
      if (sb != VGS_OK) return sb;
      hipLaunchKernelGGL(k_compress, dim3(nbV), dim3(TB), 0, c->stream, c->parent.p, V);
      compressed = true;
      vgs_status se = vgs_readback_end(c, &n_cand, 4);
      if (se != VGS_OK) return se;
    } else {
      VGS_READBACK_ON(c, s, &n_cand, d_ncand, 4);
    }
    if (n_cand > 0) {
      unsigned int* d_chg4 = (unsigned int*)(mcnt + 4);
      for (int round = 0; round < 1 << 18; ++round) {
        VGS_HIP_TRY(c, hipMemsetAsync(d_chg4, 0, 16, s));
        for (int q = 0; q < 4; ++q)
          hipLaunchKernelGGL((k_cc_pass<false>), dim3(n_cand), dim3(64), 0, s, c->work_ids.p, (int)n_cand, c->used_ids.p,
                             c->adj_key.p, c->adj_cnt.p, c->adj_mused.p, c->adj_stride, c->node.p, c->csize.p, c->cc_flags.p, MP, c->attach.p, d_chg4 + q);
        unsigned int ch = 0;
        if (hide && !united) {
          vgs_status sb = vgs_readback_begin(c, d_chg4 + 3, 4);
          if (sb != VGS_OK) return sb;
          hipLaunchKernelGGL(k_union_mutual, dim3((unsigned)((U + UM_ROWS - 1) / UM_ROWS)), dim3(64), 0, c->stream, c->used_ids.p, U, c->adj_key.p, c->adj_cnt.p,
                             c->adj_stride, mutual, c->attach.p, (const uint8_t*)nullptr, c->parent.p, 0, (const uint8_t*)nullptr, (const uint32_t*)nullptr, 0, LcGate{nullptr, 0u});
          united = true;
          vgs_status se = vgs_readback_end(c, &ch, 4);
          if (se != VGS_OK) return se;
        } else {
          VGS_READBACK_ON(c, s, &ch, d_chg4 + 3, 4);
        }
        if (!ch) break;
      }
      hipLaunchKernelGGL((k_cc_pass<true>), dim3(n_cand), dim3(64), 0, s, c->work_ids.p, (int)n_cand, c->used_ids.p, c->adj_key.p,
                         c->adj_cnt.p, c->adj_mused.p, c->adj_stride, c->node.p, c->csize.p, c->cc_flags.p, MP, c->attach.p, d_changed);
    }
    if (s != c->stream) {
      VGS_HIP_TRY(c, hipEventRecord(c->ev_join, s));
      VGS_HIP_TRY(c, hipStreamWaitEvent(c->stream, c->ev_join, 0));
    }
  } else {
    VGS_HIP_TRY(c, c->conn.ensure(16));
  }
  if (c->have_region && U == 0) { vgs_status so = vgs_compute_owned(c); if (so != VGS_OK) return so; }
  if (U > 0 && !compressed) hipLaunchKernelGGL(k_compress, dim3(nbV), dim3(TB), 0, c->stream, c->parent.p, V);
  if (U > 0 && !united)
    hipLaunchKernelGGL(k_union_mutual, dim3((unsigned)((U + UM_ROWS - 1) / UM_ROWS)), dim3(64), 0, c->stream, c->used_ids.p, U, c->adj_key.p, c->adj_cnt.p,
                       c->adj_stride, mutual, c->attach.p, c->have_region ? c->owned.p : nullptr, c->parent.p, 1, (const uint8_t*)nullptr, (const uint32_t*)nullptr, 0, LcGate{nullptr, 0u});
  else if (U > 0 && n_cand > 0)
    hipLaunchKernelGGL(k_union_attach, dim3((n_cand + TB - 1) / TB), dim3(TB), 0, c->stream, c->work_ids.p, (int)n_cand, c->used_ids.p, c->attach.p, c->parent.p,
                       c->have_region ? c->owned.p : (const uint8_t*)nullptr);
  hipLaunchKernelGGL(k_flatten, dim3(nbV), dim3(TB), 0, c->stream, c->parent.p, V, c->have_region ? c->owned.p : nullptr, c->csz.p);
  VGS_HIP_TRY(c, hipEventRecord(c->ev[14], c->stream));
  uint32_t* keep_flag = c->head_flag.p;
  VGS_HIP_TRY(c, c->head_flag.ensure(V + 1));
  keep_flag = c->head_flag.p;
  unsigned int* d_nroots = (unsigned int*)(mcnt + 2);
  hipLaunchKernelGGL(k_root_flags, dim3((unsigned)((V + 1023) / 1024)), dim3(1024), 0, c->stream, c->parent.p, c->csz.p, V, c->P.method == 3 ? -1 : c->P.voxels_min,
                     keep_flag, d_nroots);
  size_t bytes = 0;
  VGS_HIP_TRY(c, rocprim::exclusive_scan(nullptr, bytes, keep_flag, c->kept_rank.p, 0u, (size_t)V, rocprim::plus<uint32_t>(), c->stream));
  VGS_HIP_TRY(c, c->sort_tmp.ensure(bytes));
  VGS_HIP_TRY(c, rocprim::exclusive_scan(c->sort_tmp.p, bytes, keep_flag, c->kept_rank.p, 0u, (size_t)V, rocprim::plus<uint32_t>(), c->stream));
  hipLaunchKernelGGL(k_voxel_labels, dim3(nbV), dim3(TB), 0, c->stream, c->parent.p, keep_flag, c->kept_rank.p, V, c->vox_label.p,
                     (unsigned int*)(mcnt + 3));
  c->pt_labels_pending = c->have_region && N > 0;
  if (!c->pt_labels_pending)
    hipLaunchKernelGGL(k_point_labels, dim3((unsigned)((N + TB - 1) / TB)), dim3(TB), 0, c->stream, c->perm_b.p, c->pt_vox.p, c->vox_label.p,
                       N, c->pt_label.p);
  VGS_HIP_TRY(c, hipEventRecord(c->ev[15], c->stream));
  c->labels_event_valid = true;
  VGS_HIP_TRY(c, hipGetLastError());
  uint64_t hm[4] = {0, 0, 0, 0};
  VGS_READBACK(c, hm, mcnt, sizeof(hm));
  { float lms = 0.f; if (hipEventElapsedTime(&lms, c->ev[14], c->ev[15]) == hipSuccess) c->times[VGS_T_LABELS] = lms; }
  const unsigned int n_roots = (unsigned int)hm[2];
  if (U > 0 && n_cand > 0) n_succ = (unsigned int)hm[1];
  c->counts[VGS_N_REATTACHED] = n_succ;
  c->counts[VGS_N_CLUSTERS] = n_roots;
  c->counts[VGS_N_KEPT] = (int64_t)(unsigned int)hm[3];
  c->counts[VGS_N_ISOLATED] = n_cand;
  return VGS_OK;
}
```

### vgs-svgs-segmentation_amd/csrc/multigpu.hip

```cpp
#include <algorithm>
#include <cstring>
#include <vector>

#include <rocprim/rocprim.hpp>

#include "vgs_context.hpp"

__global__ void k_point_sources(const uint32_t* __restrict__ perm, const uint32_t* __restrict__ pt_vox, int64_t nf, int64_t own_first, int64_t n_own,
                                int64_t V, uint8_t* __restrict__ mix) {
  int64_t j = (int64_t)blockIdx.x * blockDim.x + threadIdx.x;
  if (j >= nf) return;
  const uint32_t v = pt_vox[j];
  const int64_t i = (int64_t)perm[j];
  if (v != 0xffffffffu) mix[((i >= own_first && i < own_first + n_own) ? 0 : V) + v] = 1;
}

__global__ void k_owned(const uint64_t* __restrict__ vox_code, int64_t V, float res_f, float min_x, float min_y, double lo_x, double lo_y,
                        double hi_x, double hi_y, uint8_t* __restrict__ owned, uint8_t* __restrict__ straddle, const uint8_t* __restrict__ mix, double near) {
  int64_t v = (int64_t)blockIdx.x * blockDim.x + threadIdx.x;
  if (v >= V) return;
  const uint64_t code = vox_code[v];
  const double cx = (double)vm_voxel_center(vm_compact21(code >> 2), res_f, min_x);
  const double cy = (double)vm_voxel_center(vm_compact21(code >> 1), res_f, min_y);
  owned[v] = (cx >= lo_x && cx < hi_x && cy >= lo_y && cy < hi_y) ? 1 : 0;
  const double h = 0.5001 * (double)res_f;
  bool st = fabs(cx - lo_x) < h || fabs(cx - hi_x) < h || fabs(cy - lo_y) < h || fabs(cy - hi_y) < h;
  if (mix) st = st || (owned[v] ? mix[V + v] != 0 : mix[v] != 0);
  const bool nr = fabs(cx - lo_x) < near || fabs(cx - hi_x) < near || fabs(cy - lo_y) < near || fabs(cy - hi_y) < near;
  straddle[v] = (uint8_t)((st ? 1 : 0) | (nr ? 2 : 0));
}

vgs_status vgs_compute_owned(vgs_ctx* c) {
  VGS_HIP_TRY(c, c->owned.ensure(c->V > 0 ? c->V : 1));
  VGS_HIP_TRY(c, c->straddle.ensure(c->V > 0 ? c->V : 1));
  if (c->V == 0) return VGS_OK;
  const uint8_t* mix = nullptr;
  if (c->n_own >= 0 && c->Nf > 0) {
    VGS_HIP_TRY(c, c->mixsrc.ensure(2 * (size_t)c->V));
    VGS_HIP_TRY(c, hipMemsetAsync(c->mixsrc.p, 0, 2 * (size_t)c->V, c->stream));
    hipLaunchKernelGGL(k_point_sources, dim3((unsigned)((c->Nf + 255) / 256)), dim3(256), 0, c->stream, c->perm_b.p, c->pt_vox.p, c->Nf, c->own_first, c->n_own, c->V, c->mixsrc.p);
    mix = c->mixsrc.p;
  }
  hipLaunchKernelGGL(k_owned, dim3((unsigned)((c->V + 255) / 256)), dim3(256), 0, c->stream, c->vox_code.p, c->V, c->P.voxel_size,
                     (float)c->box.min[0], (float)c->box.min[1], c->own_lo[0], c->own_lo[1], c->own_hi[0], c->own_hi[1], c->owned.p, c->straddle.p, mix,
                     (double)c->P.graph_size + 2.0 * (double)c->P.voxel_size);
  VGS_HIP_TRY(c, hipGetLastError());
  return VGS_OK;
}

__global__ __launch_bounds__(64) void k_boundary(const uint32_t* __restrict__ used_ids, int64_t U, const uint64_t* __restrict__ adj_key,
                                                 const uint32_t* __restrict__ adj_cnt, int adj_stride, const uint8_t* __restrict__ mutual,
                                                 const int32_t* __restrict__ attach, const uint8_t* __restrict__ owned,
                                                 const uint32_t* __restrict__ parent, const uint64_t* __restrict__ vox_code,
                                                 unsigned long long cap, unsigned long long* __restrict__ n_out,
                                                 uint64_t* __restrict__ out_code, int32_t* __restrict__ out_root, const uint8_t* __restrict__ straddle) {
  const int lane = threadIdx.x;
  const int64_t u_mine = (int64_t)blockIdx.x * 64 + lane;
  uint32_t i_mine = 0;
  bool near_mine = false, oi_mine = false;
  if (u_mine < U) { i_mine = used_ids[u_mine]; near_mine = (straddle[i_mine] & 2) != 0; oi_mine = owned[i_mine] != 0; }
  unsigned long long pub_mask = 0ull;
  unsigned long long todo = __ballot(near_mine);
  while (todo) {
    const int src = __ffsll((long long)todo) - 1;
    todo &= todo - 1ull;
    const int64_t u = (int64_t)blockIdx.x * 64 + src;
    const bool oi = __shfl((int)oi_mine, src, 64) != 0;
    const int n = (int)adj_cnt[u];
    const uint64_t* row = adj_key + u * adj_stride;
    const uint8_t* mrow = mutual + u * adj_stride;
    bool pub = false;
    for (int k = lane; k < n; k += 64) {
      const uint32_t t = (uint32_t)row[k];
      const bool ot = owned[t] != 0;
      pub = pub || (oi ? !ot : (ot && mrow[k] != 0));
    }
    if (__ballot(pub) != 0ull) pub_mask |= 1ull << src;
  }
  if (u_mine >= U) return;
  const bool pub = ((pub_mask >> lane) & 1ull) != 0ull;
  const int32_t a = attach[i_mine];
  const bool att = a >= 0 && oi_mine && !owned[a];
  const unsigned int cnt = (pub || att ? 1u : 0u) + (att ? 1u : 0u);
  if (cnt == 0) return;
  const unsigned long long p = atomicAdd(n_out, (unsigned long long)cnt);
  if (p + cnt > cap) return;
  out_code[p] = vox_code[i_mine]; out_root[p] = (int32_t)parent[i_mine];
  if (att) { out_code[p + 1] = vox_code[a]; out_root[p + 1] = (int32_t)parent[a]; }
}

__global__ void k_boundary_straddle(const uint8_t* __restrict__ straddle, int64_t V, const uint32_t* __restrict__ parent,
                                    const uint64_t* __restrict__ vox_code, unsigned long long cap, unsigned long long* __restrict__ n_out,
                                    uint64_t* __restrict__ out_code, int32_t* __restrict__ out_root) {
  int64_t v = (int64_t)blockIdx.x * blockDim.x + threadIdx.x;
  if (v >= V || !(straddle[v] & 1)) return;
  const unsigned long long p = atomicAdd(n_out, 1ull);
  if (p < cap) { out_code[p] = vox_code[v]; out_root[p] = (int32_t)parent[v]; }
}

__global__ void k_apply_root_labels(const uint32_t* __restrict__ parent, const int32_t* __restrict__ root_label, int64_t V,
                                    int32_t* __restrict__ vox_label) {
  int64_t v = (int64_t)blockIdx.x * blockDim.x + threadIdx.x;
  if (v >= V) return;
  vox_label[v] = root_label[parent[v]];
}

__global__ void k_point_labels2(const uint32_t* __restrict__ perm, const uint32_t* __restrict__ pt_vox, const int32_t* __restrict__ vox_label,
                                int64_t N, int32_t* __restrict__ label) {
  int64_t j = (int64_t)blockIdx.x * blockDim.x + threadIdx.x;
  if (j >= N) return;
  const uint32_t v = pt_vox[j];
  label[perm[j]] = (v == 0xffffffffu) ? -1 : vox_label[v];
}

__global__ void k_bnd_heads(const uint64_t* __restrict__ code_sorted, int64_t n, uint32_t* __restrict__ head) {
  int64_t k = (int64_t)blockIdx.x * blockDim.x + threadIdx.x;
  if (k < n) head[k] = (k == 0 || code_sorted[k] != code_sorted[k - 1]) ? 1u : 0u;
}

__global__ void k_bnd_compact(const uint64_t* __restrict__ code_sorted, const int32_t* __restrict__ root_sorted, const uint32_t* __restrict__ head,
                              const uint32_t* __restrict__ scan_incl, int64_t n, const uint32_t* __restrict__ csz,
                              uint64_t* __restrict__ out_code, int32_t* __restrict__ out_root, int32_t* __restrict__ out_cnt,
                              uint8_t* __restrict__ broot) {
  int64_t k = (int64_t)blockIdx.x * blockDim.x + threadIdx.x;
  if (k >= n || !head[k]) return;
  const uint32_t pos = scan_incl[k] - 1u;
  const int32_t r = root_sorted[k];
  out_code[pos] = code_sorted[k];
  out_root[pos] = r;
  out_cnt[pos] = (int32_t)csz[r];
  broot[r] = 1;
}

__global__ void k_local_kept_flags(const uint32_t* __restrict__ parent, const uint32_t* __restrict__ csz, const uint8_t* __restrict__ broot,
                                   int64_t V, int voxels_min, uint32_t* __restrict__ flag) {
  int64_t v = (int64_t)blockIdx.x * blockDim.x + threadIdx.x;
  if (v >= V) return;
  flag[v] = (parent[v] == (uint32_t)v && !broot[v] && (int)csz[v] > voxels_min) ? 1u : 0u;
}

__global__ void k_tile_root_labels(const uint32_t* __restrict__ flag, const uint32_t* __restrict__ rank_excl, int64_t V, int32_t local_base,
                                   int32_t* __restrict__ root_label) {
  int64_t v = (int64_t)blockIdx.x * blockDim.x + threadIdx.x;
  if (v >= V) return;
  root_label[v] = flag[v] ? local_base + (int32_t)rank_excl[v] : -1;
}

__global__ void k_scatter_labels(const int32_t* __restrict__ root, const int32_t* __restrict__ label, int64_t n, int64_t V,
                                 int32_t* __restrict__ root_label, unsigned int* __restrict__ bad) {
  int64_t k = (int64_t)blockIdx.x * blockDim.x + threadIdx.x;
  if (k >= n) return;
  const int32_t r = root[k];
  if (r < 0 || r >= V) { atomicOr(bad, 1u); return; }
  root_label[r] = label[k];
}

__global__ __launch_bounds__(256) void k_points_bbox(const float* __restrict__ xyz, int stride_f, int64_t n, float* __restrict__ out,
                                                     unsigned long long* __restrict__ n_finite) {
  __shared__ float s_v[6][4];
  __shared__ unsigned long long s_n[4];
  float lo[3] = {3.0e38f, 3.0e38f, 3.0e38f}, hi[3] = {-3.0e38f, -3.0e38f, -3.0e38f};
  unsigned long long cnt = 0;
  for (int64_t i = (int64_t)blockIdx.x * blockDim.x + threadIdx.x; i < n; i += (int64_t)gridDim.x * blockDim.x) {
    const float* p = xyz + i * stride_f;
    const float x = p[0], y = p[1], z = p[2];
    const bool fin = (vm_bits(x) & 0x7f800000u) != 0x7f800000u && (vm_bits(y) & 0x7f800000u) != 0x7f800000u && (vm_bits(z) & 0x7f800000u) != 0x7f800000u;
    if (fin) {
      lo[0] = fminf(lo[0], x); lo[1] = fminf(lo[1], y); lo[2] = fminf(lo[2], z);
      hi[0] = fmaxf(hi[0], x); hi[1] = fmaxf(hi[1], y); hi[2] = fmaxf(hi[2], z);
      ++cnt;
    }
  }
  for (int o = 32; o > 0; o >>= 1) {
    for (int a = 0; a < 3; ++a) { lo[a] = fminf(lo[a], __shfl_xor(lo[a], o, 64)); hi[a] = fmaxf(hi[a], __shfl_xor(hi[a], o, 64)); }
    cnt += __shfl_xor(cnt, o, 64);
  }
  const int lane = threadIdx.x & 63, wave = threadIdx.x >> 6;
  if (lane == 0) { for (int a = 0; a < 3; ++a) { s_v[a][wave] = lo[a]; s_v[3 + a][wave] = hi[a]; } s_n[wave] = cnt; }
  __syncthreads();
  if (threadIdx.x == 0) {
    for (int a = 0; a < 3; ++a) {
      out[6 * blockIdx.x + a] = fminf(fminf(s_v[a][0], s_v[a][1]), fminf(s_v[a][2], s_v[a][3]));
      out[6 * blockIdx.x + 3 + a] = fmaxf(fmaxf(s_v[3 + a][0], s_v[3 + a][1]), fmaxf(s_v[3 + a][2], s_v[3 + a][3]));
    }
    atomicAdd(n_finite, s_n[0] + s_n[1] + s_n[2] + s_n[3]);
  }
}

extern "C" {

vgs_status vgs_points_bbox(vgs_ctx* c, float* bbox6, int64_t* n_finite) {
  if (!c || !bbox6 || !n_finite) return VGS_E_ARG;
  if (c->stage < ST_POINTS) { c->err = "vgs_points_bbox: no input cloud"; return VGS_E_STATE; }
  VGS_HIP_TRY(c, hipSetDevice(c->device));
  *n_finite = 0;
// ... 132 lines not shown
                       c->vox_code.p, cap, d_n, c->bnd_code.p, c->bnd_root.p);
    unsigned long long n = 0;
    VGS_HIP_TRY(c, hipMemcpyAsync(&n, d_n, 8, hipMemcpyDeviceToHost, c->stream));
    VGS_HIP_TRY(c, hipStreamSynchronize(c->stream));
    if (n <= cap) {
      *n_records = (int64_t)n;
      if (code && n) VGS_HIP_TRY(c, hipMemcpy(code, c->bnd_code.p, n * 8, hipMemcpyDeviceToHost));
      if (root && n) VGS_HIP_TRY(c, hipMemcpy(root, c->bnd_root.p, n * 4, hipMemcpyDeviceToHost));
      return VGS_OK;
    }
    cap = n + 1024;
  }
  c->err = "vgs_get_boundary: record buffer overflow";
  return VGS_E_NOMEM;
}

vgs_status vgs_get_boundary_roots(vgs_ctx* c, int64_t* n_records, uint64_t* code, int32_t* root, int32_t* owned_voxels, int64_t* n_kept_local) {
  if (!c || !n_records) return VGS_E_ARG;
  if (c->stage < ST_SEGMENTED || !c->have_region) { c->err = "vgs_get_boundary_roots: segment a context with an owned region first"; return VGS_E_STATE; }
  VGS_HIP_TRY(c, hipSetDevice(c->device));
  const int64_t V = c->V;
  const int TB = 256;
  if (!code || c->bnd_unique < 0) {
    int64_t n_raw = 0;
    vgs_status st = vgs_get_boundary(c, &n_raw, nullptr, nullptr);
    if (st != VGS_OK) return st;
    VGS_HIP_TRY(c, c->broot.ensure(V > 0 ? V : 1));
    VGS_HIP_TRY(c, hipMemsetAsync(c->broot.p, 0, V > 0 ? V : 1, c->stream));
    int64_t n_unique = 0;
    if (n_raw > 0) {
      const size_t n = (size_t)n_raw;
      VGS_HIP_TRY(c, c->bnd_code2.ensure(2 * n)); VGS_HIP_TRY(c, c->bnd_root2.ensure(2 * n)); VGS_HIP_TRY(c, c->bnd_cnt.ensure(n));
      VGS_HIP_TRY(c, c->head_flag.ensure(n + 1)); VGS_HIP_TRY(c, c->kept_rank.ensure(n + 1));
      uint64_t* code_sorted = c->bnd_code2.p + n;
      int32_t* root_sorted = c->bnd_root2.p + n;
      size_t sort_bytes = 0, scan_bytes = 0;
      VGS_HIP_TRY(c, rocprim::radix_sort_pairs(nullptr, sort_bytes, c->bnd_code.p, code_sorted, c->bnd_root.p, root_sorted, n, 0, 64, c->stream));
      VGS_HIP_TRY(c, rocprim::inclusive_scan(nullptr, scan_bytes, c->head_flag.p, c->kept_rank.p, n, rocprim::plus<uint32_t>(), c->stream));
      VGS_HIP_TRY(c, c->sort_tmp.ensure(std::max(sort_bytes, scan_bytes)));
      VGS_HIP_TRY(c, rocprim::radix_sort_pairs(c->sort_tmp.p, sort_bytes, c->bnd_code.p, code_sorted, c->bnd_root.p, root_sorted, n, 0, 64, c->stream));
      hipLaunchKernelGGL(k_bnd_heads, dim3((unsigned)((n + TB - 1) / TB)), dim3(TB), 0, c->stream, code_sorted, (int64_t)n, c->head_flag.p);
      VGS_HIP_TRY(c, rocprim::inclusive_scan(c->sort_tmp.p, scan_bytes, c->head_flag.p, c->kept_rank.p, n, rocprim::plus<uint32_t>(), c->stream));
      hipLaunchKernelGGL(k_bnd_compact, dim3((unsigned)((n + TB - 1) / TB)), dim3(TB), 0, c->stream, code_sorted, root_sorted, c->head_flag.p,
                         c->kept_rank.p, (int64_t)n, c->csz.p, c->bnd_code2.p, c->bnd_root2.p, c->bnd_cnt.p, c->broot.p);
      uint32_t last = 0;
      VGS_HIP_TRY(c, hipMemcpyAsync(&last, c->kept_rank.p + (n - 1), 4, hipMemcpyDeviceToHost, c->stream));
      VGS_HIP_TRY(c, hipStreamSynchronize(c->stream));
      n_unique = (int64_t)last;
    }
    int64_t kept_local = 0;
    if (V > 0) {
      VGS_HIP_TRY(c, c->head_flag.ensure(V + 1)); VGS_HIP_TRY(c, c->kept_rank.ensure(V + 1));
      hipLaunchKernelGGL(k_local_kept_flags, dim3((unsigned)((V + TB - 1) / TB)), dim3(TB), 0, c->stream, c->parent.p, c->csz.p, c->broot.p, V,
                         c->P.voxels_min, c->head_flag.p);
      size_t scan_bytes = 0;
      VGS_HIP_TRY(c, rocprim::exclusive_scan(nullptr, scan_bytes, c->head_flag.p, c->kept_rank.p, 0u, (size_t)V, rocprim::plus<uint32_t>(), c->stream));
      VGS_HIP_TRY(c, c->sort_tmp.ensure(scan_bytes));
      VGS_HIP_TRY(c, rocprim::exclusive_scan(c->sort_tmp.p, scan_bytes, c->head_flag.p, c->kept_rank.p, 0u, (size_t)V, rocprim::plus<uint32_t>(), c->stream));
      uint32_t last_rank = 0, last_flag = 0;
      VGS_HIP_TRY(c, hipMemcpyAsync(&last_rank, c->kept_rank.p + (V - 1), 4, hipMemcpyDeviceToHost, c->stream));
      VGS_HIP_TRY(c, hipMemcpyAsync(&last_flag, c->head_flag.p + (V - 1), 4, hipMemcpyDeviceToHost, c->stream));
      VGS_HIP_TRY(c, hipStreamSynchronize(c->stream));
      kept_local = (int64_t)last_rank + last_flag;
    }
    VGS_HIP_TRY(c, hipGetLastError());
    c->bnd_unique = n_unique;
    c->bnd_kept_local = kept_local;
  }
  *n_records = c->bnd_unique;
  if (n_kept_local) *n_kept_local = c->bnd_kept_local;
  const size_t n = (size_t)c->bnd_unique;
  if (code && n) VGS_HIP_TRY(c, hipMemcpy(code, c->bnd_code2.p, n * 8, hipMemcpyDeviceToHost));
  if (root && n) VGS_HIP_TRY(c, hipMemcpy(root, c->bnd_root2.p, n * 4, hipMemcpyDeviceToHost));
  if (owned_voxels && n) VGS_HIP_TRY(c, hipMemcpy(owned_voxels, c->bnd_cnt.p, n * 4, hipMemcpyDeviceToHost));
  return VGS_OK;
}

vgs_status vgs_apply_tile_labels(vgs_ctx* c, int32_t local_base, const int32_t* root, const int32_t* label, int64_t n_roots) {
  if (c) { c->cl_valid = false; c->sd_valid = false; c->sb_valid[0] = c->sb_valid[1] = false; c->sg_valid = false; c->cmp_valid = false; c->rf_valid = false; c->cmp_own_cells = -1; c->sg_halo_valid = false; c->sg_own_K = -1; c->rf_halo_valid = false; c->rf_band_n = -1; }
  if (!c || (n_roots > 0 && (!root || !label))) return VGS_E_ARG;
  if (c->stage < ST_SEGMENTED || c->bnd_unique < 0) { c->err = "vgs_apply_tile_labels: vgs_get_boundary_roots first"; return VGS_E_STATE; }
  VGS_HIP_TRY(c, hipSetDevice(c->device));
  if (c->d2h_open && c->d2h_src == c->pt_label.p) { VGS_HIP_TRY(c, hipEventSynchronize(c->ev_d2h)); c->d2h_open = false; }
  const int64_t V = c->V, N = c->N;
  if (V == 0) return VGS_OK;
  const int TB = 256;
  VGS_HIP_TRY(c, c->root_label.ensure(V));
  hipLaunchKernelGGL(k_tile_root_labels, dim3((unsigned)((V + TB - 1) / TB)), dim3(TB), 0, c->stream, c->head_flag.p, c->kept_rank.p, V, local_base,
                     c->root_label.p);
  if (n_roots > 0) {
    VGS_HIP_TRY(c, c->bnd_root2.ensure(2 * (size_t)n_roots + 2)); VGS_HIP_TRY(c, c->counters.ensure(64));
    int32_t* d_root = c->bnd_root2.p;
    int32_t* d_label = c->bnd_root2.p + n_roots;
    unsigned int* d_bad = (unsigned int*)(c->counters.p + 33);
    VGS_HIP_TRY(c, hipMemsetAsync(d_bad, 0, 4, c->stream));
    VGS_HIP_TRY(c, hipMemcpyAsync(d_root, root, (size_t)n_roots * 4, hipMemcpyHostToDevice, c->stream));
    VGS_HIP_TRY(c, hipMemcpyAsync(d_label, label, (size_t)n_roots * 4, hipMemcpyHostToDevice, c->stream));
    hipLaunchKernelGGL(k_scatter_labels, dim3((unsigned)((n_roots + TB - 1) / TB)), dim3(TB), 0, c->stream, d_root, d_label, n_roots, V,
                       c->root_label.p, d_bad);
    unsigned int bad = 0;
    VGS_HIP_TRY(c, hipMemcpyAsync(&bad, d_bad, 4, hipMemcpyDeviceToHost, c->stream));
    VGS_HIP_TRY(c, hipStreamSynchronize(c->stream));
    if (bad) { c->err = "vgs_apply_tile_labels: root out of range"; return VGS_E_ARG; }
  }
  hipLaunchKernelGGL(k_apply_root_labels, dim3((unsigned)((V + TB - 1) / TB)), dim3(TB), 0, c->stream, c->parent.p, c->root_label.p, V,
                     c->vox_label.p);
  hipLaunchKernelGGL(k_point_labels2, dim3((unsigned)((N + TB - 1) / TB)), dim3(TB), 0, c->stream, c->perm_b.p, c->pt_vox.p, c->vox_label.p, N,
                     c->pt_label.p);
  c->pt_labels_pending = false;
  VGS_HIP_TRY(c, hipEventRecord(c->ev[15], c->stream));
  c->labels_event_valid = true;
  VGS_HIP_TRY(c, hipGetLastError());
  VGS_HIP_TRY(c, hipStreamSynchronize(c->stream));
  c->bnd_unique = -1;
  return VGS_OK;
}

vgs_status vgs_get_owned_roots(vgs_ctx* c, int64_t* n_roots, int32_t* root, int32_t* owned_voxels) {
  if (!c || !n_roots) return VGS_E_ARG;
  if (c->stage < ST_SEGMENTED) { c->err = "vgs_get_owned_roots: segment first"; return VGS_E_STATE; }
  VGS_HIP_TRY(c, hipSetDevice(c->device));
  std::vector<uint32_t> par((size_t)c->V), csz((size_t)c->V);
  if (c->V > 0) {
    VGS_HIP_TRY(c, hipMemcpy(par.data(), c->parent.p, par.size() * 4, hipMemcpyDeviceToHost));
    VGS_HIP_TRY(c, hipMemcpy(csz.data(), c->csz.p, csz.size() * 4, hipMemcpyDeviceToHost));
  }
  int64_t n = 0;
  for (int64_t v = 0; v < c->V; ++v)
    if (par[v] == (uint32_t)v && csz[v] > 0) {
      if (root) root[n] = (int32_t)v;
      if (owned_voxels) owned_voxels[n] = (int32_t)csz[v];
      ++n;
    }
  *n_roots = n;
  return VGS_OK;
}

vgs_status vgs_apply_root_labels(vgs_ctx* c, const int32_t* root, const int32_t* label, int64_t n_roots) {
  if (c) { c->cl_valid = false; c->sd_valid = false; c->sb_valid[0] = c->sb_valid[1] = false; c->sg_valid = false; c->cmp_valid = false; c->rf_valid = false; c->cmp_own_cells = -1; c->sg_halo_valid = false; c->sg_own_K = -1; c->rf_halo_valid = false; c->rf_band_n = -1; }
  if (!c || (n_roots > 0 && (!root || !label))) return VGS_E_ARG;
  if (c->stage < ST_SEGMENTED) { c->err = "vgs_apply_root_labels: segment first"; return VGS_E_STATE; }
  VGS_HIP_TRY(c, hipSetDevice(c->device));
  if (c->d2h_open && c->d2h_src == c->pt_label.p) { VGS_HIP_TRY(c, hipEventSynchronize(c->ev_d2h)); c->d2h_open = false; }
  const int64_t V = c->V, N = c->N;
  if (V == 0) return VGS_OK;
  std::vector<int32_t> map((size_t)V, -1);
  for (int64_t k = 0; k < n_roots; ++k) {
    if (root[k] < 0 || root[k] >= V) { c->err = "vgs_apply_root_labels: root out of range"; return VGS_E_ARG; }
    map[root[k]] = label[k];
  }
  VGS_HIP_TRY(c, c->root_label.ensure(V));
  VGS_HIP_TRY(c, hipMemcpy(c->root_label.p, map.data(), (size_t)V * 4, hipMemcpyHostToDevice));
  const int TB = 256;
  hipLaunchKernelGGL(k_apply_root_labels, dim3((unsigned)((V + TB - 1) / TB)), dim3(TB), 0, c->stream, c->parent.p, c->root_label.p, V,
                     c->vox_label.p);
  hipLaunchKernelGGL(k_point_labels2, dim3((unsigned)((N + TB - 1) / TB)), dim3(TB), 0, c->stream, c->perm_b.p, c->pt_vox.p, c->vox_label.p, N,
                     c->pt_label.p);
  c->pt_labels_pending = false;
  VGS_HIP_TRY(c, hipEventRecord(c->ev[15], c->stream));
  c->labels_event_valid = true;
  VGS_HIP_TRY(c, hipGetLastError());
  VGS_HIP_TRY(c, hipStreamSynchronize(c->stream));
  return VGS_OK;
}

}
```

### vgs-svgs-segmentation_amd/csrc/svgs.hip

```cpp
#include <cstring>
#include <string.h>

#include <rocprim/rocprim.hpp>

#include <algorithm>
#include <cmath>
#include <vector>

#include "vgs_context.hpp"

#define SV_ROW 512

__global__ void k_sv_keys(const int32_t* __restrict__ label, int64_t n, int32_t max_label, const float* __restrict__ xyz, int stride_f,
                          uint32_t* __restrict__ key, uint32_t* __restrict__ perm) {
  int64_t i = (int64_t)blockIdx.x * blockDim.x + threadIdx.x;
  if (i >= n) return;
  const int32_t l = label[i];
  const float* p = xyz + i * stride_f;
  const bool finite = isfinite(p[0]) && isfinite(p[1]) && isfinite(p[2]);
  key[i] = (finite && l > 0 && l < max_label) ? (uint32_t)l : 0xffffffffu;
  perm[i] = (uint32_t)i;
}

__global__ void k_sv_heads(const uint32_t* __restrict__ key, int64_t n, uint32_t* __restrict__ head) {
  int64_t j = (int64_t)blockIdx.x * blockDim.x + threadIdx.x;
  if (j >= n) return;
  const uint32_t k = key[j];
  head[j] = (k != 0xffffffffu && (j == 0 || key[j - 1] != k)) ? 1u : 0u;
}

__global__ void k_sv_count_valid(const uint32_t* __restrict__ key, int64_t n, unsigned long long* __restrict__ n_valid) {
  int64_t lo = 0, hi = n;
  while (lo < hi) { int64_t mid = (lo + hi) >> 1; if (key[mid] != 0xffffffffu) lo = mid + 1; else hi = mid; }
  *n_valid = (unsigned long long)lo;
}

__global__ void k_sv_table(const uint32_t* __restrict__ key, const uint32_t* __restrict__ head, const uint32_t* __restrict__ scan, int64_t n,
                           uint32_t* __restrict__ pt_vox, uint32_t* __restrict__ vox_start, uint64_t* __restrict__ vox_code) {
  int64_t j = (int64_t)blockIdx.x * blockDim.x + threadIdx.x;
  if (j >= n) return;
  const uint32_t k = key[j];
  if (k == 0xffffffffu) { pt_vox[j] = 0xffffffffu; return; }
  const uint32_t s = scan[j] - 1u;
  pt_vox[j] = s;
  if (head[j]) { vox_start[s] = (uint32_t)j; vox_code[s] = (uint64_t)k; }
}

__global__ void k_sv_gather(const float* __restrict__ xyz, int stride_f, const uint32_t* __restrict__ perm, int64_t nf,
                            float* __restrict__ xs, float* __restrict__ ys, float* __restrict__ zs) {
  int64_t j = (int64_t)blockIdx.x * blockDim.x + threadIdx.x;
  if (j >= nf) return;
  const float* p = xyz + (int64_t)perm[j] * stride_f;
  xs[j] = p[0]; ys[j] = p[1]; zs[j] = p[2];
}

__global__ void k_sv_set(uint32_t* p, uint32_t v) { *p = v; }

vgs_status vgs_stage_svgs_group(vgs_ctx* c) {
  const int64_t N = c->N;
  c->V = 0; c->Nf = 0; c->U = 0;
  if (N == 0) { c->counts[VGS_N_FINITE] = 0; c->counts[VGS_N_VOXELS] = 0; c->counts[VGS_N_SUPERVOXELS] = 0; return VGS_OK; }
  VGS_HIP_TRY(c, c->sv_key_a.ensure(N)); VGS_HIP_TRY(c, c->sv_key_b.ensure(N));
  VGS_HIP_TRY(c, c->perm_a.ensure(N)); VGS_HIP_TRY(c, c->perm_b.ensure(N));
  VGS_HIP_TRY(c, c->head_flag.ensure(N)); VGS_HIP_TRY(c, c->pt_vox.ensure(N));
  VGS_HIP_TRY(c, c->counters.ensure(64));
  const int TB = 256;
  const unsigned nb = (unsigned)((N + TB - 1) / TB);
  hipLaunchKernelGGL(k_sv_keys, dim3(nb), dim3(TB), 0, c->stream, c->sv_label.p, N, c->sv_max_label, c->xyz, c->stride_f, c->sv_key_a.p,
                     c->perm_a.p);
  size_t sort_bytes = 0, scan_bytes = 0;
  VGS_HIP_TRY(c, rocprim::radix_sort_pairs(nullptr, sort_bytes, c->sv_key_a.p, c->sv_key_b.p, c->perm_a.p, c->perm_b.p, (size_t)N, 0, 32, c->stream));
  VGS_HIP_TRY(c, rocprim::inclusive_scan(nullptr, scan_bytes, c->head_flag.p, c->perm_a.p, (size_t)N, rocprim::plus<uint32_t>(), c->stream));
  VGS_HIP_TRY(c, c->sort_tmp.ensure(std::max(sort_bytes, scan_bytes)));
  VGS_HIP_TRY(c, rocprim::radix_sort_pairs(c->sort_tmp.p, sort_bytes, c->sv_key_a.p, c->sv_key_b.p, c->perm_a.p, c->perm_b.p, (size_t)N, 0, 32, c->stream));
  unsigned long long* d_cnt = (unsigned long long*)c->counters.p;
  hipLaunchKernelGGL(k_sv_heads, dim3(nb), dim3(TB), 0, c->stream, c->sv_key_b.p, N, c->head_flag.p);
  hipLaunchKernelGGL(k_sv_count_valid, dim3(1), dim3(1), 0, c->stream, c->sv_key_b.p, N, d_cnt);
  uint32_t* scan = c->perm_a.p;
  VGS_HIP_TRY(c, rocprim::inclusive_scan(c->sort_tmp.p, scan_bytes, c->head_flag.p, scan, (size_t)N, rocprim::plus<uint32_t>(), c->stream));
  unsigned long long nf = 0;
  uint32_t s_total = 0;
  VGS_HIP_TRY(c, hipMemcpyAsync(&nf, d_cnt, 8, hipMemcpyDeviceToHost, c->stream));
  VGS_HIP_TRY(c, hipMemcpyAsync(&s_total, scan + (N - 1), 4, hipMemcpyDeviceToHost, c->stream));
  VGS_HIP_TRY(c, hipStreamSynchronize(c->stream));
  c->Nf = (int64_t)nf;
  c->V = (int64_t)s_total;
  VGS_HIP_TRY(c, c->vox_code.ensure(c->V + 1)); VGS_HIP_TRY(c, c->vox_start.ensure(c->V + 1));
  hipLaunchKernelGGL(k_sv_table, dim3(nb), dim3(TB), 0, c->stream, c->sv_key_b.p, c->head_flag.p, scan, N, c->pt_vox.p, c->vox_start.p,
                     c->vox_code.p);
  hipLaunchKernelGGL(k_sv_set, dim3(1), dim3(1), 0, c->stream, c->vox_start.p + c->V, (uint32_t)c->Nf);
  VGS_HIP_TRY(c, c->xs.ensure(c->Nf + 1)); VGS_HIP_TRY(c, c->ys.ensure(c->Nf + 1)); VGS_HIP_TRY(c, c->zs.ensure(c->Nf + 1));
  if (c->Nf > 0)
    hipLaunchKernelGGL(k_sv_gather, dim3((unsigned)((c->Nf + TB - 1) / TB)), dim3(TB), 0, c->stream, c->xyz, c->stride_f, c->perm_b.p, c->Nf,
                       c->xs.p, c->ys.p, c->zs.p);
  VGS_HIP_TRY(c, hipGetLastError());
  c->counts[VGS_N_FINITE] = c->Nf;
  c->counts[VGS_N_VOXELS] = c->V;
  c->counts[VGS_N_SUPERVOXELS] = c->V;
  return VGS_OK;
}

#define SV_OFF (1 << 20)
__device__ __forceinline__ uint64_t sv_cell_code(int cx, int cy, int cz) {
  return ((uint64_t)(uint32_t)(cx + SV_OFF) << 42) | ((uint64_t)(uint32_t)(cy + SV_OFF) << 21) | (uint64_t)(uint32_t)(cz + SV_OFF);
}
__device__ __forceinline__ uint32_t sv_hash_slot(uint64_t code, uint32_t hbits) {
  return (uint32_t)((code * 0x9E3779B97F4A7C15ull) >> (64 - hbits));
}

__global__ void k_sv_cells(const NodeRec* __restrict__ node, int64_t S, double cell, uint64_t* __restrict__ code, uint32_t* __restrict__ id) {
  int64_t s = (int64_t)blockIdx.x * blockDim.x + threadIdx.x;
  if (s >= S) return;
  const int cx = (int)floor((double)node[s].c[0] / cell), cy = (int)floor((double)node[s].c[1] / cell), cz = (int)floor((double)node[s].c[2] / cell);
  code[s] = sv_cell_code(cx, cy, cz);
  id[s] = (uint32_t)s;
}

__global__ void k_sv_cell_heads(const uint64_t* __restrict__ code, int64_t S, uint32_t* __restrict__ head) {
  int64_t j = (int64_t)blockIdx.x * blockDim.x + threadIdx.x;
  if (j >= S) return;
  head[j] = (j == 0 || code[j - 1] != code[j]) ? 1u : 0u;
}

__global__ void k_sv_cell_table(const uint64_t* __restrict__ code, const uint32_t* __restrict__ head, const uint32_t* __restrict__ scan, int64_t S,
                                uint32_t* __restrict__ cell_start, unsigned long long* __restrict__ hkey, uint32_t* __restrict__ hval,
                                uint32_t hbits) {
  int64_t j = (int64_t)blockIdx.x * blockDim.x + threadIdx.x;
  if (j >= S || !head[j]) return;
  const uint32_t cidx = scan[j] - 1u;
  cell_start[cidx] = (uint32_t)j;
  const unsigned long long key = code[j] + 1ull;
  const uint32_t mask = (1u << hbits) - 1u;
  uint32_t s = sv_hash_slot(key, hbits);
  while (true) {
    unsigned long long prev = atomicCAS(&hkey[s], 0ull, key);
    if (prev == 0ull) { hval[s] = cidx; return; }
    s = (s + 1) & mask;
  }
}

__global__ __launch_bounds__(64) void k_sv_neighbours(const NodeRec* __restrict__ node, int64_t S, double cell, float r2,
                                                      const uint64_t* __restrict__ hkey, const uint32_t* __restrict__ hval, uint32_t hbits,
                                                      const uint32_t* __restrict__ cell_start, const uint32_t* __restrict__ sorted_id,
// ... 109 lines not shown
```

### vgs-svgs-segmentation_amd/csrc/vgs_context.hpp

```cpp
#ifndef VGS_CONTEXT_HPP_
#define VGS_CONTEXT_HPP_

#include <hip/hip_runtime.h>
#include <stdint.h>
#include <string.h>

#include <string>
#include <vector>

#include "../../include/vgs.h"
#include "vgs_math.h"
#include "pairlist.hpp"

typedef VgsNode NodeRec;
static_assert(sizeof(NodeRec) == 64, "NodeRec must be 64 bytes");

#ifdef __HIPCC__
__device__ __forceinline__ int64_t vgs_xcd_item(unsigned int b, int64_t n) {
  const int64_t per = (n + 7) >> 3;
  return (int64_t)(b & 7u) * per + (int64_t)(b >> 3);
}
#endif
static inline unsigned int vgs_xcd_grid(int64_t n) { return (unsigned int)(((n + 7) >> 3) << 3); }

template <typename T>
struct DevBuf {
  T* p = nullptr;
  size_t cap = 0;
  hipError_t ensure(size_t n) {
    if (n <= cap) return hipSuccess;
    if (p) { hipError_t e = hipFree(p); if (e != hipSuccess) return e; p = nullptr; cap = 0; }
    size_t want = n + n / 8 + 64;
    hipError_t e = hipMalloc((void**)&p, want * sizeof(T));
    if (e != hipSuccess) return e;
    cap = want;
    return hipSuccess;
  }
  void release() { if (p) (void)hipFree(p); p = nullptr; cap = 0; }
};

struct OctreeBox {
  double min[3] = {0, 0, 0}, max[3] = {0, 0, 0};
  double res = 0;
  int depth = 0;
  bool defined = false;
  uint64_t shift[3] = {0, 0, 0};
  bool contains(const float* p) const;
  void adopt(const float* p);
};

struct Epoch {
  int64_t first;
  double min[3];
  uint64_t shift[3];
};

#define VGS_MAX_EPOCHS 96

struct SgRec {
  double w_sum;
  uint32_t cnt_lt, n_finite;
  int32_t a, b;
  float w_min, w_max;
};
struct SgPart {
  double w_sum;
  int64_t n_pairs, n_finite;
  int32_t nodes_a, nodes_b;
  float w_min, w_max;
};

enum Stage { ST_NONE = 0, ST_POINTS = 1, ST_VOXELS = 2, ST_FEATURES = 3, ST_ADJACENCY = 4, ST_SEGMENTED = 5 };

struct VgsKnobs {
  int a1_max = 4;
  float shell0 = 8.0f;
  float cap_frac = 0.7f;
  int dbg_stop = 0;
  int max_rounds = 6;
  int dbg_max_m = 0;
  int dbg_xl_from = 0;
  int near_min_own = 7;
  int fv_blocks = 512;
  int only_class = -1;
  bool no_dense = false;
  bool no_overlap = false;
  bool no_near = false;
  bool no_adjmasks = false;
  int vote_period = 64;
  int cross_lds_kb = 0;
  bool no_sort32 = false;
  bool no_pg_xl = false;
  bool no_connbits = false;
  bool no_pairlists = false;
  bool no_vote = false;
  int vote_force = 0;
  int ho_grid = -1;
  int pg_min_frac = 8;
  int pg_wide = 1;
  int pg_wide_frac = 8;
  bool debug = false;
};

struct vgs_ctx {
  vgs_params P;
  VgsKnobs K;
  int device = 0;
  hipStream_t stream = nullptr;
  hipStream_t stream2 = nullptr;
  hipStream_t stream3 = nullptr;
  hipStream_t stream4 = nullptr;
  std::string err;
  int stage = ST_NONE;
  void* pin = nullptr;

  const float* xyz = nullptr;
  DevBuf<float> xyz_buf[2];
  int xyz_cur = 0;
  hipStream_t s_h2d = nullptr, s_d2h = nullptr;
  hipEvent_t ev_h2d = nullptr, ev_d2h = nullptr;
  hipEvent_t ev_rb = nullptr;
  bool gathered = false;
  bool bricks_ready = false;
  bool staged = false;
  int64_t staged_n = 0;
  int staged_stride = 12;
  bool pt_labels_pending = false;
  bool labels_event_valid = false;
  bool d2h_open = false;
  const int32_t* d2h_src = nullptr;
  int64_t N = 0;
  int stride_f = 3;

  OctreeBox box;
  bool grid_pinned = false;
  bool grid_covers = false;
  int n_epochs = 0;

  DevBuf<uint64_t> code_a, code_b;
  DevBuf<uint32_t> perm_a, perm_b;
  DevBuf<uint8_t> sort_tmp;
  DevBuf<uint64_t> grow_state;
  DevBuf<uint32_t> pt_vox;
  DevBuf<uint32_t> vox_tile;
  DevBuf<uint32_t> head_flag;
  DevBuf<uint64_t> vox_code;
  DevBuf<uint32_t> vox_start;
  DevBuf<float> xs, ys, zs;
  int64_t Nf = 0;
  int64_t V = 0;
  int code_bits = 0;

  DevBuf<NodeRec> node;
  DevBuf<uint32_t> used_ids, used_rank;
  int64_t U = 0;

  DevBuf<uint64_t> hkey;
  DevBuf<uint32_t> hval;
  uint32_t hbits = 0;
  DevBuf<int32_t> offsets;
  DevBuf<uint64_t> adj_masks;
  int adj_mask_nb = 0;
  bool adj_tab_valid = false;
  float adj_tab_graph = 0.f, adj_tab_voxel = 0.f;
  DevBuf<uint16_t> adj_gtab;
  DevBuf<int32_t> adj_nvals;
  DevBuf<uint8_t> adj_nrank;
  int adj_ngroups = 0, adj_gstride = 0;
  bool adj_have_gtab = false;
  int n_off = 0;
  int adj_R = 0;
  int adj_stride = 0;
  DevBuf<uint64_t> adj_key;
  DevBuf<uint16_t> adj_off;
  bool adj_have_off = false;
  DevBuf<uint32_t> conn_bits;
  int cb_words = 0, cb_R = 0;
  bool cb_enabled = false;
  DevBuf<uint32_t> adj_cnt, adj_mused;
  bool adj_pruned = false;
  float adj_r2 = 0.f;

  DevBuf<uint8_t> nl_cnt;
  DevBuf<uint32_t> nl_tot;
  DevBuf<float4> nl_ent;
  bool nl_enabled = false;
  int nl_reach_steps = 0;
  bool nl_direct = false;

  DevBuf<uint8_t> pl_state;
  DevBuf<float4> pl_ent;
  DevBuf<uint32_t> pl_work;
  bool pl_enabled = false;
  bool pl_enabled_at_launch = false;
  hipEvent_t ev_ho = nullptr, ev_ho2 = nullptr;
  hipEvent_t ev_fork = nullptr, ev_join = nullptr;
  float pl_w_ring = 0.0f;

  DevBuf<uint8_t> conn;
  DevBuf<uint32_t> evals;
  DevBuf<uint8_t> lc_pending;
  DevBuf<uint8_t> lc_defer_flag;
  DevBuf<uint32_t> lc_defer;
  struct { bool open = false; bool dense = true; bool gated = false;  bool many = false;  unsigned int grid_f = 0, grid_g = 0, nabc[5] = {0, 0, 0, 0, 0}; float tail_ms = 0.f; bool pg_xl_queued = false;  bool rb_queued = false;  } lc_tail;
  int64_t lc_diag[16] = {0};
  DevBuf<float> lc_ctab;
  float lc_ctab_key[8] = {0}, lc_ctab_scale = 0.0f;
  bool lc_ctab_valid = false;
  DevBuf<uint32_t> csize;
  DevBuf<int32_t> attach;
  DevBuf<uint8_t> cc_flags;
  DevBuf<uint32_t> parent;
  DevBuf<uint32_t> csz, kept_rank;
  DevBuf<int32_t> vox_label;
  DevBuf<int32_t> pt_label;
  DevBuf<int32_t> pt_label_alt;
  DevBuf<int64_t> cl_off;
  DevBuf<int32_t> cl_idx;
  bool cl_valid = false;
  DevBuf<uint32_t> sd_key, sd_ids, sd_vp, sd_seg;
  DevBuf<uint8_t> sd_tmp;
  DevBuf<double> sd_part;
  DevBuf<int64_t> sd_npts;
  DevBuf<int32_t> sd_nnodes;
  DevBuf<float> sd_bbox, sd_eig8;
  DevBuf<double> sd_cen, sd_cov, sd_eval, sd_evec;
// ... 141 lines not shown
}
#endif
#define VGS_READBACK(ctx, dst, src, bytes) do { vgs_status _s = vgs_readback((ctx), (dst), (src), (bytes)); if (_s != VGS_OK) return _s; } while (0)
#define VGS_READBACK_ON(ctx, s, dst, src, bytes) do { vgs_status _s = vgs_readback_on((ctx), (s), (dst), (src), (bytes)); if (_s != VGS_OK) return _s; } while (0)

static inline vgs_status vgs_readback_begin(vgs_ctx* c, const void* src_dev, size_t bytes) {
  if (bytes > 2048 || !c->pin || !c->ev_rb) return VGS_E_ARG;
  VGS_HIP_TRY(c, hipMemcpyAsync((char*)c->pin + 2048, src_dev, bytes, hipMemcpyDeviceToHost, c->stream));
  VGS_HIP_TRY(c, hipEventRecord(c->ev_rb, c->stream));
  return VGS_OK;
}
static inline vgs_status vgs_readback_end(vgs_ctx* c, void* dst, size_t bytes) {
  VGS_HIP_TRY(c, hipEventSynchronize(c->ev_rb));
  memcpy(dst, (char*)c->pin + 2048, bytes);
  return VGS_OK;
}
static inline bool vgs_can_split_readback(const vgs_ctx* c) { return c->pin != nullptr && c->ev_rb != nullptr; }

#define SD_TB 256
#define SD_PPT 8
#define SD_CHUNK (SD_TB * SD_PPT)
struct SdPrep { uint32_t *ids, *vp, *seg_node, *seg_chunk; int64_t n_chunks_max; };
vgs_status sd_prepare(vgs_ctx* c, int64_t K, SdPrep& o);
vgs_status sd_own_anchor(vgs_ctx* c, int64_t K, const SdPrep& P);
static inline bool vgs_is_tile(const vgs_ctx* c) { return c->have_region || c->n_own >= 0; }
#ifdef __HIPCC__
__device__ __forceinline__ int64_t vgs_find_voxel(const uint64_t* __restrict__ vox_code, int64_t V, uint64_t q) {
  int64_t lo = 0, hi = V;
  while (lo < hi) { const int64_t mid = (lo + hi) >> 1; if (vox_code[mid] > q) lo = mid + 1; else hi = mid; }
  return (lo < V && vox_code[lo] == q) ? lo : V;
}
struct SdChunk { uint32_t k, n0, a, b, m; };
__device__ __forceinline__ bool sd_walk(const uint32_t* __restrict__ vox_start, const uint32_t* __restrict__ ids, const uint32_t* __restrict__ vp,
                                        const uint32_t* __restrict__ seg_node, const uint32_t* __restrict__ seg_chunk, uint32_t K,
                                        uint32_t* __restrict__ s_vp, uint32_t* __restrict__ s_dl, SdChunk& o) {
  const uint32_t c = blockIdx.x;
  o.k = 0xffffffffu;
  if (c >= seg_chunk[K]) return false;
  uint32_t lo = 0, hi = K - 1;
  while (lo < hi) { const uint32_t mid = (lo + hi + 1) >> 1; if (seg_chunk[mid] <= c) lo = mid; else hi = mid - 1; }
  const uint32_t k = lo;
  o.k = k;
  const uint32_t n0 = seg_node[k], n1 = seg_node[k + 1];
  const uint32_t a = vp[n0] + (c - seg_chunk[k]) * SD_CHUNK;
  const uint32_t b = min(a + SD_CHUNK, vp[n1]);
  if (n1 <= n0 || a >= b) return false;
  uint32_t i0 = n0, i1 = n1 - 1;
  while (i0 < i1) { const uint32_t mid = (i0 + i1 + 1) >> 1; if (vp[mid] <= a) i0 = mid; else i1 = mid - 1; }
  uint32_t j0 = i0 + 1, j1 = n1;
  while (j0 < j1) { const uint32_t mid = (j0 + j1) >> 1; if (vp[mid] < b) j0 = mid + 1; else j1 = mid; }
  const uint32_t m = min(j0 - i0, (uint32_t)SD_CHUNK);
  for (uint32_t t = threadIdx.x; t < m; t += SD_TB) {
    const uint32_t i = i0 + t, q = vp[i];
    s_vp[t] = q;
    s_dl[t] = vox_start[ids[i]] - q;
  }
  o.n0 = n0; o.a = a; o.b = b; o.m = m;
  return true;
}
__device__ __forceinline__ uint32_t sd_pos(const uint32_t* __restrict__ s_vp, const uint32_t* __restrict__ s_dl, uint32_t m, uint32_t q) {
  uint32_t l = 0, h = m - 1;
  while (l < h) { const uint32_t mid = (l + h + 1) >> 1; if (s_vp[mid] <= q) l = mid; else h = mid - 1; }
  return q + s_dl[l];
}
#endif

vgs_status vgs_cut_order(vgs_ctx* c, std::vector<uint16_t>& ord_host, std::vector<uint32_t>& k_host, bool want_lists = false,
                         const uint8_t* list_flag = nullptr, std::vector<uint32_t>* list_cnt = nullptr, std::vector<int32_t>* list_ids = nullptr);
void vgs_read_env_knobs(vgs_ctx* c);

vgs_status vgs_stage_voxelize(vgs_ctx* c);
vgs_status vgs_stage_features(vgs_ctx* c);
vgs_status vgs_stage_adjacency(vgs_ctx* c);
vgs_status vgs_run_adjacency(vgs_ctx* c, bool full, uint64_t* out_key, uint32_t* out_cnt, uint32_t* out_nall, float r2, const uint32_t* ids = nullptr,
                             int64_t n_ids = 0);
bool vgs_unused_are_inert(const vgs_params& p);
vgs_status vgs_stage_nearlists(vgs_ctx* c);
vgs_status vgs_pairlists_begin(vgs_ctx* c, hipStream_t strm);
vgs_status vgs_pairlists_build(vgs_ctx* c, hipStream_t strm, const uint32_t* const* ids, const unsigned int* const* n_dev, const unsigned int* n_host,
                               int n_lists, bool all_rows, const float* ctab, float ctab_scale, float d2_stop, int slot, const LcGate& gate,
                               bool big_rows_too);
vgs_status vgs_stage_localcut(vgs_ctx* c);
vgs_status vgs_ensure_point_labels(vgs_ctx* c);
vgs_status vgs_localcut_finish_queue(vgs_ctx* c, hipStream_t s);
vgs_status vgs_localcut_finish(vgs_ctx* c, hipStream_t s, unsigned int* n_deferred);
vgs_status vgs_stage_merge(vgs_ctx* c);
vgs_status vgs_clusters_on_device(vgs_ctx* c);
vgs_status vgs_segdesc_on_device(vgs_ctx* c);
vgs_status vgs_segbox_on_device(vgs_ctx* c, int frame);
void sb_launch_frames(vgs_ctx* c, const double* evec, const double* cov, int64_t K, int frame, double* out);
vgs_status vgs_check_label_range(vgs_ctx* c, const char* fn, const int32_t* labels_dev, int64_t n, int64_t K);
vgs_status vgs_upload_point_labels(vgs_ctx* c, const int32_t* labels_host, int64_t n, const int32_t** labels_dev);
vgs_status vgs_seggraph_on_device(vgs_ctx* c);
vgs_status vgs_halo_find(vgs_ctx* c, const uint64_t* code_dev, const int32_t* label_dev, int64_t n, int32_t* halo_dev);
vgs_status vgs_refine_on_device(vgs_ctx* c, const vgs_refine_params& rp, int64_t* counts4);
vgs_status vgs_refine_own_on_device(vgs_ctx* c, const vgs_refine_params& rp, int64_t* counts5);
vgs_status vgs_stage_vccs(vgs_ctx* c);
vgs_status vgs_stage_svgs_group(vgs_ctx* c);
vgs_status vgs_stage_svgs_neighbours(vgs_ctx* c);
vgs_status vgs_grow_box_from(vgs_ctx* c, OctreeBox& box, bool record_epochs);
vgs_status vgs_compute_owned(vgs_ctx* c);

#endif
```

### vgs-svgs-segmentation_amd/csrc/voxelize.hip

```cpp
#include <cstddef>
#include <cstdlib>
#include <cstring>
#include <string.h>

#include <rocprim/rocprim.hpp>

#include <algorithm>
#include <cmath>
#include <limits>

#include "vgs_context.hpp"

bool OctreeBox::contains(const float* p) const {
  if (!defined) return false;
  for (int a = 0; a < 3; ++a)
    if ((double)p[a] < min[a] || (double)p[a] >= max[a]) return false;
  return true;
}

void OctreeBox::adopt(const float* p) {
  const double eps = (double)std::numeric_limits<float>::epsilon();
  while (true) {
    if (!defined) {
      for (int a = 0; a < 3; ++a) { min[a] = (double)p[a] - res / 2; max[a] = (double)p[a] + res / 2; }
// ... 362 lines not shown
    return VGS_OK;
  }
  const int pinned = (c->grid_pinned && record_epochs) ? 1 : 0;
  const int blocks = (int)std::max<int64_t>(8, std::min<int64_t>((c->N / 4 + 255) / 256 + 1, (int64_t)c->K.fv_blocks));
  hipLaunchKernelGGL(k_grow_prefix, dim3(1), dim3(1024), 0, c->stream, c->xyz, c->stride_f, std::min<int64_t>(c->N, 8192), d_g, pinned);
  for (int batch = 0; batch < 64; ++batch) {
    for (int k = 0; k < (batch == 0 ? 2 : 8); ++k) {
      hipLaunchKernelGGL(k_first_violation, dim3(blocks), dim3(256), 0, c->stream, c->xyz, c->stride_f, c->N, d_g);
      hipLaunchKernelGGL(k_adopt, dim3(1), dim3(1), 0, c->stream, c->xyz, c->stride_f, d_g, pinned);
    }
    VGS_READBACK(c, &h, d_g, offsetof(GrowState, epochs));
    if (h.done) break;
  }
  if (h.done == 2) { c->err = "a point lies outside the pinned grid"; return VGS_E_ARG; }
  if (h.overflow || !h.done) { c->err = "octree grew more than VGS_MAX_EPOCHS times"; return VGS_E_UNSUPPORTED; }
  for (int a = 0; a < 3; ++a) { box.min[a] = h.min[a]; box.max[a] = h.max[a]; box.shift[a] = h.shift[a]; }
  box.depth = h.depth; box.defined = h.defined != 0;
  if (record_epochs) c->n_epochs = h.n_epochs;
  return VGS_OK;
}

static vgs_status grow_box(vgs_ctx* c) {
  if (!c->grid_pinned) {
    c->box = OctreeBox();
    c->box.res = (double)c->P.voxel_size;
  }
  return vgs_grow_box_from(c, c->box, true);
}

template <typename KeyT>
static vgs_status voxelize_sorted_table(vgs_ctx* c) {
  const int64_t N = c->N;
  const int TB = 256;
  const unsigned nb = (unsigned)((N + TB - 1) / TB);
  KeyT* code_a = (KeyT*)c->code_a.p;
  KeyT* code_b = (KeyT*)c->code_b.p;
  const unsigned key_bits = (unsigned)(c->code_bits + 1);
  int idx_bits = 1;
  while (idx_bits < 32 && ((int64_t)1 << idx_bits) < N) ++idx_bits;
  const int pack_shift = (sizeof(KeyT) == 8 && (int)key_bits + idx_bits <= 64) ? idx_bits : 0;
  hipLaunchKernelGGL((k_make_codes<KeyT>), dim3(nb), dim3(TB), 0, c->stream, c->xyz, c->stride_f, N, (const GrowState*)c->grow_state.p, c->box.res,
                     c->code_bits, code_a, c->perm_a.p, pack_shift);

  using nine_bits = rocprim::radix_sort_config<rocprim::default_config, rocprim::default_config,
                                               rocprim::radix_sort_onesweep_config<rocprim::kernel_config<1024, 6>, rocprim::kernel_config<1024, 6>, 9,
                                                                                   rocprim::block_radix_rank_algorithm::match>>;
  const bool use9 = (key_bits + 8) / 9 < (key_bits + 7) / 8;
  auto sort_pairs = [&](void* tmp, size_t& bytes) -> hipError_t {
    if (pack_shift > 0)
      return use9 ? rocprim::radix_sort_keys_desc<nine_bits>(tmp, bytes, code_a, code_b, (size_t)N, (unsigned)pack_shift, (unsigned)pack_shift + key_bits, c->stream)
                  : rocprim::radix_sort_keys_desc(tmp, bytes, code_a, code_b, (size_t)N, (unsigned)pack_shift, (unsigned)pack_shift + key_bits, c->stream);
    return use9 ? rocprim::radix_sort_pairs_desc<nine_bits>(tmp, bytes, code_a, code_b, c->perm_a.p, c->perm_b.p, (size_t)N, 0, key_bits, c->stream)
                : rocprim::radix_sort_pairs_desc(tmp, bytes, code_a, code_b, c->perm_a.p, c->perm_b.p, (size_t)N, 0, key_bits, c->stream);
  };
  size_t tmp_bytes = 0;
  VGS_HIP_TRY(c, sort_pairs(nullptr, tmp_bytes));
  VGS_HIP_TRY(c, c->sort_tmp.ensure(tmp_bytes));
  VGS_HIP_TRY(c, sort_pairs(c->sort_tmp.p, tmp_bytes));
  const int64_t n_tiles = (N + VR_TILE - 1) / VR_TILE;
  VGS_HIP_TRY(c, c->vox_tile.ensure((size_t)(2 * n_tiles)));
  uint32_t* tile_heads = c->vox_tile.p;
  uint32_t* tile_valid = c->vox_tile.p + n_tiles;
  unsigned long long* d_cnt = (unsigned long long*)c->counters.p;
  hipLaunchKernelGGL((k_run_counts<KeyT>), dim3((unsigned)n_tiles), dim3(VR_TB), 0, c->stream, code_b, N, pack_shift, c->perm_b.p, tile_heads, tile_valid);
  hipLaunchKernelGGL(k_tile_offsets, dim3(1), dim3(1024), 0, c->stream, tile_heads, tile_valid, n_tiles, d_cnt);
  unsigned long long h2[2] = {0, 0};
  if (vgs_can_split_readback(c)) {
    { vgs_status sb = vgs_readback_begin(c, d_cnt, sizeof(h2)); if (sb != VGS_OK) return sb; }
    VGS_HIP_TRY(c, c->xs.ensure(N + 1)); VGS_HIP_TRY(c, c->ys.ensure(N + 1)); VGS_HIP_TRY(c, c->zs.ensure(N + 1));
    hipLaunchKernelGGL(k_gather_points, dim3(nb), dim3(TB), 0, c->stream, c->xyz, c->stride_f, c->perm_b.p, N, c->xs.p, c->ys.p, c->zs.p);
    c->gathered = true;
    { vgs_status se = vgs_readback_end(c, h2, sizeof(h2)); if (se != VGS_OK) return se; }
  } else {
    VGS_READBACK(c, h2, d_cnt, sizeof(h2));
  }
  const unsigned long long nf = h2[0];
  const uint32_t v_total = (uint32_t)h2[1];
  c->Nf = (int64_t)nf;
  c->V = (int64_t)v_total;
  VGS_HIP_TRY(c, c->vox_code.ensure(c->V + 1)); VGS_HIP_TRY(c, c->vox_start.ensure(c->V + 1));
  const uint64_t mask = (c->code_bits >= 64) ? ~0ull : ((1ull << c->code_bits) - 1ull);
  hipLaunchKernelGGL((k_voxel_runs<KeyT>), dim3((unsigned)n_tiles), dim3(VR_TB), 0, c->stream, code_b, N, pack_shift, tile_heads, mask, c->pt_vox.p,
                     c->vox_code.p, c->vox_start.p, v_total, (uint32_t)c->Nf);
  return VGS_OK;
}

vgs_status vgs_stage_voxelize(vgs_ctx* c) {
  const int64_t N = c->N;
  c->V = 0; c->Nf = 0; c->U = 0;
  vgs_status st = grow_box(c);
  if (st != VGS_OK) return st;
  if (c->n_epochs == 0) {
    c->counts[VGS_N_FINITE] = 0; c->counts[VGS_N_VOXELS] = 0; c->counts[VGS_N_DEPTH] = 0;
    return VGS_OK;
  }
  if (c->box.depth > 21) { c->err = "octree depth > 21 (64-bit voxel codes exhausted)"; return VGS_E_UNSUPPORTED; }
  c->code_bits = 3 * c->box.depth;

  VGS_HIP_TRY(c, c->code_a.ensure(N)); VGS_HIP_TRY(c, c->code_b.ensure(N));
  VGS_HIP_TRY(c, c->perm_a.ensure(N)); VGS_HIP_TRY(c, c->perm_b.ensure(N));
  VGS_HIP_TRY(c, c->pt_vox.ensure(N));
  const int TB = 256;
  c->gathered = false;
  st = (c->code_bits + 1 <= 32) ? voxelize_sorted_table<uint32_t>(c) : voxelize_sorted_table<uint64_t>(c);
  if (st != VGS_OK) return st;
  if (!c->gathered) { VGS_HIP_TRY(c, c->xs.ensure(c->Nf + 1)); VGS_HIP_TRY(c, c->ys.ensure(c->Nf + 1)); VGS_HIP_TRY(c, c->zs.ensure(c->Nf + 1)); }
  if (c->Nf > 0 && !c->gathered) {
    const unsigned nbf = (unsigned)((c->Nf + TB - 1) / TB);
    hipLaunchKernelGGL(k_gather_points, dim3(nbf), dim3(TB), 0, c->stream, c->xyz, c->stride_f, c->perm_b.p, c->Nf, c->xs.p, c->ys.p,
                       c->zs.p);
  }
  VGS_HIP_TRY(c, hipGetLastError());
  c->counts[VGS_N_FINITE] = c->Nf;
  c->counts[VGS_N_VOXELS] = c->V;
  c->counts[VGS_N_DEPTH] = c->box.depth;
  return VGS_OK;
}
```

Before: 1.688 billion.

## Precompute input-order point-to-voxel map on side stream during localcut

```diff
diff --git a/vgs-svgs-segmentation_amd/csrc/brick_table.hpp b/vgs-svgs-segmentation_amd/csrc/brick_table.hpp
--- a/vgs-svgs-segmentation_amd/csrc/brick_table.hpp
+++ b/vgs-svgs-segmentation_amd/csrc/brick_table.hpp
@@ -69,6 +69,22 @@
   return (int)(table[s].first + (uint32_t)__popcll(above));
 }
 
+__device__ __forceinline__ uint32_t brick_find_code(const Brick* __restrict__ table, uint32_t hbits, uint64_t code) {
+  const unsigned long long key = brick_key(vm_compact21(code >> 2), vm_compact21(code >> 1), vm_compact21(code));
+  const uint32_t mask = (1u << hbits) - 1u;
+  uint32_t s = hash_slot(key, hbits);
+  while (true) {
+    const unsigned long long k = table[s].key;
+    if (k == key) break;
+    if (k == 0ull) return 0xffffffffu;
+    s = (s + 1) & mask;
+  }
+  const unsigned long long occ = table[s].occ;
+  const int local = (int)(code & 63ull);
+  if (!((occ >> local) & 1ull)) return 0xffffffffu;
+  const unsigned long long above = (local == 63) ? 0ull : (occ >> (local + 1));
+  return table[s].first + (uint32_t)__popcll(above);
+}
 
 static __global__ void k_brick_clear(Brick* __restrict__ table, size_t H) {
   const size_t e = (size_t)blockIdx.x * blockDim.x + threadIdx.x;
@@ -87,6 +103,7 @@
   VGS_HIP_TRY(c, c->hkey.ensure(H * (sizeof(Brick) / 8)));
   hipLaunchKernelGGL(k_brick_clear, dim3((unsigned)((H + 255) / 256)), dim3(256), 0, c->stream, (Brick*)c->hkey.p, H);
   hipLaunchKernelGGL(k_brick_insert, dim3((unsigned)((V + 255) / 256)), dim3(256), 0, c->stream, c->vox_code.p, node, V, (Brick*)c->hkey.p, hbits);
+  c->bricks_current = true;
   return VGS_OK;
 }
 
diff --git a/vgs-svgs-segmentation_amd/csrc/capi.hip b/vgs-svgs-segmentation_amd/csrc/capi.hip
--- a/vgs-svgs-segmentation_amd/csrc/capi.hip
+++ b/vgs-svgs-segmentation_amd/csrc/capi.hip
@@ -70,6 +70,7 @@
   k.dbg_stop = geti("VGS_DBG_STOP", k.dbg_stop); k.max_rounds = geti("VGS_ROUNDS", k.max_rounds); k.dbg_max_m = geti("VGS_DBG_MAXM", k.dbg_max_m); k.dbg_xl_from = geti("VGS_DBG_XL_FROM", k.dbg_xl_from);
   k.near_min_own = geti("VGS_NEARMINOWN", k.near_min_own); k.fv_blocks = geti("VGS_FV_BLOCKS", k.fv_blocks); k.only_class = geti("VGS_ONLY_CLASS", k.only_class);
   k.no_dense = has("VGS_NO_DENSE"); k.no_overlap = has("VGS_NO_OVERLAP"); k.no_near = has("VGS_NO_NEAR"); k.no_adjmasks = has("VGS_NO_ADJMASKS"); k.no_connbits = has("VGS_NO_CONNBITS"); k.no_pg_xl = has("VGS_NO_PG_XL"); k.no_sort32 = has("VGS_NO_SORT32"); k.no_pairlists = has("VGS_NO_PAIRLISTS"); k.no_vote = has("VGS_NO_VOTE"); k.vote_force = geti("VGS_VOTE_FORCE", 0); k.cross_lds_kb = geti("VGS_CROSS_LDS", k.cross_lds_kb); { int vp = geti("VGS_VOTE_PERIOD", k.vote_period); if (vp >= 2 && vp <= 4096 && (vp & (vp - 1)) == 0) k.vote_period = vp; } k.pg_wide = geti("VGS_PG_WIDE", k.pg_wide); k.pg_wide_frac = geti("VGS_PG_WIDEFRAC", k.pg_wide_frac); k.pg_min_frac = geti("VGS_PG_MINFRAC", k.pg_min_frac); k.ho_grid = geti("VGS_HO_GRID", k.ho_grid);
+  k.pvi_grid = geti("VGS_PVI_GRID", k.pvi_grid); k.pvi_scatter = has("VGS_PVI_SCATTER");
   k.debug = has("VGS_DEBUG");
 }
 
@@ -180,7 +181,8 @@
             hipEventCreateWithFlags(&c->ev_ho, hipEventDisableTiming) == hipSuccess &&
             hipEventCreateWithFlags(&c->ev_ho2, hipEventDisableTiming) == hipSuccess &&
             hipEventCreateWithFlags(&c->ev_fork, hipEventDisableTiming) == hipSuccess &&
-            hipEventCreateWithFlags(&c->ev_join, hipEventDisableTiming) == hipSuccess;
+            hipEventCreateWithFlags(&c->ev_join, hipEventDisableTiming) == hipSuccess &&
+            hipEventCreateWithFlags(&c->ev_pvi, hipEventDisableTiming) == hipSuccess;
   for (int i = 0; ok && i < 16; ++i) ok = hipEventCreate(&c->ev[i]) == hipSuccess;
   for (int i = 0; ok && i < VGS_T_COUNT; ++i) ok = hipEventCreate(&c->tev[i][0]) == hipSuccess && hipEventCreate(&c->tev[i][1]) == hipSuccess;
   if (!ok) { g_create_err = "vgs_create: hipStreamCreate/hipEventCreate failed"; vgs_destroy(c); return VGS_E_HIP; }
@@ -192,6 +194,7 @@
 void vgs_destroy(vgs_ctx* c) {
   if (!c) return;
   (void)hipSetDevice(c->device);
+  if (c->pvi_state == PVI_QUEUED) (void)hipEventSynchronize(c->ev_pvi);
   if (c->stream) (void)hipStreamSynchronize(c->stream);
   if (c->stream2) (void)hipStreamSynchronize(c->stream2);
   if (c->stream3) (void)hipStreamSynchronize(c->stream3);
@@ -200,7 +203,7 @@
   if (c->s_d2h) (void)hipStreamSynchronize(c->s_d2h);
   c->xyz_buf[0].release(); c->xyz_buf[1].release(); c->pt_label_alt.release(); c->grow_state.release();
   c->code_a.release(); c->code_b.release(); c->perm_a.release(); c->perm_b.release(); c->sort_tmp.release();
-  c->head_flag.release(); c->pt_vox.release(); c->vox_tile.release(); c->vox_code.release(); c->vox_start.release();
+  c->head_flag.release(); c->pt_vox.release(); c->pt_vox_in.release(); c->vox_tile.release(); c->vox_code.release(); c->vox_start.release();
   c->xs.release(); c->ys.release(); c->zs.release();
   c->node.release(); c->used_ids.release(); c->used_rank.release();
   c->hkey.release(); c->hval.release(); c->offsets.release(); c->adj_masks.release(); c->adj_gtab.release(); c->adj_nvals.release(); c->adj_nrank.release(); c->adj_key.release(); c->adj_off.release(); c->adj_cnt.release(); c->adj_mused.release();
@@ -244,6 +247,7 @@
   if (c->ev_ho2) (void)hipEventDestroy(c->ev_ho2);
   if (c->ev_fork) (void)hipEventDestroy(c->ev_fork);
   if (c->ev_join) (void)hipEventDestroy(c->ev_join);
+  if (c->ev_pvi) (void)hipEventDestroy(c->ev_pvi);
   if (c->ev_d2h) (void)hipEventDestroy(c->ev_d2h);
   delete c;
 }
@@ -276,6 +280,7 @@
 static vgs_status set_points_common(vgs_ctx* c, int64_t n, int32_t stride_bytes) {
   if (n < 0 || (stride_bytes != 12 && stride_bytes != 16)) { c->err = "set_points: n >= 0 and stride_bytes 12 or 16 required"; return VGS_E_ARG; }
   if (n >= (int64_t)1 << 31) { c->err = "set_points: more than 2^31-1 points"; return VGS_E_UNSUPPORTED; }
+  { vgs_status sr = vgs_point_voxel_in_reset(c); if (sr != VGS_OK) return sr; }
   c->N = n;
   c->stride_f = stride_bytes / 4;
   c->stage = ST_POINTS;
@@ -553,10 +558,10 @@
     for (int64_t j = 0; j < c->N; ++j) out[j] = -1;
     return VGS_OK;
   }
-  std::vector<uint32_t> perm((size_t)c->N), pv((size_t)c->N);
-  VGS_HIP_TRY(c, hipMemcpy(perm.data(), c->perm_b.p, perm.size() * 4, hipMemcpyDeviceToHost));
-  VGS_HIP_TRY(c, hipMemcpy(pv.data(), c->pt_vox.p, pv.size() * 4, hipMemcpyDeviceToHost));
-  for (int64_t j = 0; j < c->N; ++j) out[perm[j]] = (pv[j] == 0xffffffffu) ? -1 : (int32_t)pv[j];
+  VGS_HIP_TRY(c, hipSetDevice(c->device));
+  { vgs_status sr = vgs_point_voxel_in_ready(c, true, nullptr); if (sr != VGS_OK) return sr; }
+  VGS_HIP_TRY(c, hipMemcpyAsync(out, c->pt_vox_in.p, (size_t)c->N * 4, hipMemcpyDeviceToHost, c->stream));
+  VGS_HIP_TRY(c, hipStreamSynchronize(c->stream));
   return VGS_OK;
 }
 
diff --git a/vgs-svgs-segmentation_amd/csrc/clusters.hip b/vgs-svgs-segmentation_amd/csrc/clusters.hip
--- a/vgs-svgs-segmentation_amd/csrc/clusters.hip
+++ b/vgs-svgs-segmentation_amd/csrc/clusters.hip
@@ -34,6 +34,7 @@
     return VGS_OK;
   }
   VGS_HIP_TRY(c, c->code_a.ensure((size_t)nf)); VGS_HIP_TRY(c, c->code_b.ensure((size_t)nf));
+  c->pvi_keys = false;
   uint32_t* key_in = (uint32_t*)c->code_a.p;
   uint32_t* key_out = key_in + nf;
   uint32_t* val_out = (uint32_t*)c->cl_idx.p;
diff --git a/vgs-svgs-segmentation_amd/csrc/localcut.hip b/vgs-svgs-segmentation_amd/csrc/localcut.hip
--- a/vgs-svgs-segmentation_amd/csrc/localcut.hip
+++ b/vgs-svgs-segmentation_amd/csrc/localcut.hip
@@ -936,6 +936,7 @@
 #undef LW_LAUNCH_1W
   }
   VGS_HIP_TRY(c, hipEventRecord(c->ev[11], c->stream));
+  if (c->P.method == 2 && !c->K.no_overlap) { vgs_status sq = vgs_point_voxel_in_queue(c, c->stream3); if (sq != VGS_OK) return sq; }
   const unsigned int nab = nabc[0] + nabc[1] + nabc[4] + nabc[6];
   unsigned int grid_f = std::min<unsigned int>(nab, std::min<unsigned int>(GRID_F, nab / 32 + 256));
   if (c->K.ho_grid != 0) {
diff --git a/vgs-svgs-segmentation_amd/csrc/merge.hip b/vgs-svgs-segmentation_amd/csrc/merge.hip
--- a/vgs-svgs-segmentation_amd/csrc/merge.hip
+++ b/vgs-svgs-segmentation_amd/csrc/merge.hip
@@ -1,3 +1,4 @@
+#include <algorithm>
 #include <cstring>
 #include <string.h>
 #include <utility>
@@ -5,6 +6,7 @@
 #include <rocprim/rocprim.hpp>
 
 #include "vgs_context.hpp"
+#include "brick_table.hpp"
 
 struct MgParams {
   VgsWeightParams W;
@@ -410,14 +412,118 @@
   label[perm[j]] = (v == 0xffffffffu) ? -1 : vox_label[v];
 }
 
+__global__ __launch_bounds__(256) void k_point_voxel_in(const uint32_t* __restrict__ perm, const uint32_t* __restrict__ pt_vox, int64_t N,
+                                                        uint32_t* __restrict__ pt_vox_in) {
+  const int64_t step = (int64_t)gridDim.x * blockDim.x * 4;
+  for (int64_t j0 = ((int64_t)blockIdx.x * blockDim.x + threadIdx.x) * 4; j0 < N; j0 += step) {
+    if (j0 + 4 <= N) {
+      const uint4 p = *(const uint4*)(perm + j0), v = *(const uint4*)(pt_vox + j0);
+      pt_vox_in[p.x] = v.x; pt_vox_in[p.y] = v.y; pt_vox_in[p.z] = v.z; pt_vox_in[p.w] = v.w;
+    } else {
+      for (int64_t j = j0; j < N; ++j) pt_vox_in[perm[j]] = pt_vox[j];
+    }
+  }
+}
+
+typedef uint32_t pl_u4 __attribute__((ext_vector_type(4)));
+typedef int32_t pl_i4 __attribute__((ext_vector_type(4)));
+template <typename KeyT>
+__device__ __forceinline__ uint32_t pvi_voxel_of(KeyT k, int key_shift, uint64_t mask, const Brick* __restrict__ table, uint32_t hbits) {
+  const uint64_t c = (uint64_t)k >> key_shift;
+  return c == 0 ? 0xffffffffu : brick_find_code(table, hbits, c & mask);
+}
+template <typename KeyT>
+__global__ __launch_bounds__(256) void k_point_voxel_keys(const KeyT* __restrict__ key, int key_shift, uint64_t mask, const Brick* __restrict__ table,
+                                                          uint32_t hbits, int64_t N, uint32_t* __restrict__ pt_vox_in) {
+  typedef KeyT K4 __attribute__((ext_vector_type(4)));
+  const int64_t step = (int64_t)gridDim.x * blockDim.x * 4;
+  for (int64_t i0 = ((int64_t)blockIdx.x * blockDim.x + threadIdx.x) * 4; i0 < N; i0 += step) {
+    if (i0 + 4 <= N) {
+      const K4 k = __builtin_nontemporal_load((const K4*)(key + i0));
+      const pl_u4 o = {pvi_voxel_of<KeyT>(k.x, key_shift, mask, table, hbits), pvi_voxel_of<KeyT>(k.y, key_shift, mask, table, hbits),
+                       pvi_voxel_of<KeyT>(k.z, key_shift, mask, table, hbits), pvi_voxel_of<KeyT>(k.w, key_shift, mask, table, hbits)};
+      *(pl_u4*)(pt_vox_in + i0) = o;
+    } else {
+      for (int64_t i = i0; i < N; ++i) pt_vox_in[i] = pvi_voxel_of<KeyT>(key[i], key_shift, mask, table, hbits);
+    }
+  }
+}
+
+__device__ __forceinline__ int32_t pl_lookup(const int32_t* __restrict__ vox_label, uint32_t v) { return v == 0xffffffffu ? -1 : vox_label[v]; }
+__global__ __launch_bounds__(256) void k_point_labels_in(const uint32_t* __restrict__ pt_vox_in, const int32_t* __restrict__ vox_label, int64_t N,
+                                                         int32_t* __restrict__ label) {
+  const int64_t i0 = ((int64_t)blockIdx.x * blockDim.x + threadIdx.x) * 4;
+  if (i0 + 4 <= N) {
+    const pl_u4 v = __builtin_nontemporal_load((const pl_u4*)(pt_vox_in + i0));
+    const pl_i4 o = {pl_lookup(vox_label, v.x), pl_lookup(vox_label, v.y), pl_lookup(vox_label, v.z), pl_lookup(vox_label, v.w)};
+    __builtin_nontemporal_store(o, (pl_i4*)(label + i0));
+  } else {
+    for (int64_t i = i0; i < N; ++i) label[i] = pl_lookup(vox_label, pt_vox_in[i]);
+  }
+}
+
+vgs_status vgs_point_voxel_in_reset(vgs_ctx* c) {
+  if (c->pvi_state == PVI_QUEUED) VGS_HIP_TRY(c, hipEventSynchronize(c->ev_pvi));
+  c->pvi_state = PVI_ABSENT;
+  c->pvi_keys = false; c->bricks_current = false;
+  return VGS_OK;
+}
+
+static vgs_status pvi_launch(vgs_ctx* c, hipStream_t s, unsigned int grid) {
+  VGS_HIP_TRY(c, c->pt_vox_in.ensure((size_t)c->N));
+  if (c->pvi_keys && c->bricks_current && !c->K.pvi_scatter) {
+    const uint64_t mask = (c->code_bits >= 64) ? ~0ull : ((1ull << c->code_bits) - 1ull);
+    if (c->pvi_key_bytes == 4)
+      hipLaunchKernelGGL((k_point_voxel_keys<uint32_t>), dim3(grid), dim3(256), 0, s, (const uint32_t*)c->code_a.p, c->pvi_key_shift, mask,
+                         (const Brick*)c->hkey.p, c->hbits, c->N, c->pt_vox_in.p);
+    else
+      hipLaunchKernelGGL((k_point_voxel_keys<uint64_t>), dim3(grid), dim3(256), 0, s, (const uint64_t*)c->code_a.p, c->pvi_key_shift, mask,
+                         (const Brick*)c->hkey.p, c->hbits, c->N, c->pt_vox_in.p);
+  } else {
+    hipLaunchKernelGGL(k_point_voxel_in, dim3(grid), dim3(256), 0, s, c->perm_b.p, c->pt_vox.p, c->N, c->pt_vox_in.p);
+  }
+  return VGS_OK;
+}
+
+vgs_status vgs_point_voxel_in_queue(vgs_ctx* c, hipStream_t s) {
+  if (c->pvi_state != PVI_ABSENT || c->N <= 0 || c->Nf <= 0 || c->K.pvi_grid <= 0) return VGS_OK;
+  { vgs_status sl = pvi_launch(c, s, (unsigned int)std::min<int64_t>(c->K.pvi_grid, (c->N + 1023) / 1024)); if (sl != VGS_OK) return sl; }
+  VGS_HIP_TRY(c, hipEventRecord(c->ev_pvi, s));
+  c->pvi_state = PVI_QUEUED;
+  return VGS_OK;
+}
+
+vgs_status vgs_point_voxel_in_ready(vgs_ctx* c, bool make_absent, bool* ready) {
+  if (ready) *ready = false;
+  if (c->N <= 0 || c->Nf <= 0) return VGS_OK;
+  if (c->pvi_state == PVI_QUEUED) VGS_HIP_TRY(c, hipStreamWaitEvent(c->stream, c->ev_pvi, 0));
+  else if (c->pvi_state == PVI_ABSENT) {
+    if (!make_absent) return VGS_OK;
+    vgs_status sl = pvi_launch(c, c->stream, (unsigned int)((c->N + 1023) / 1024));
+    if (sl != VGS_OK) return sl;
+  }
+  c->pvi_state = PVI_READY;
+  if (ready) *ready = true;
+  return VGS_OK;
+}
+
+vgs_status vgs_write_point_labels(vgs_ctx* c, bool make_absent, int32_t* label) {
+  if (c->N <= 0) return VGS_OK;
+  bool ready = false;
+  { vgs_status sr = vgs_point_voxel_in_ready(c, make_absent, &ready); if (sr != VGS_OK) return sr; }
+  if (ready)
+    hipLaunchKernelGGL(k_point_labels_in, dim3((unsigned)((c->N + 1023) / 1024)), dim3(256), 0, c->stream, c->pt_vox_in.p, c->vox_label.p, c->N, label);
+  else
+    hipLaunchKernelGGL(k_point_labels, dim3((unsigned)((c->N + 255) / 256)), dim3(256), 0, c->stream, c->perm_b.p, c->pt_vox.p, c->vox_label.p, c->N, label);
+  return VGS_OK;
+}
+
 vgs_status vgs_ensure_point_labels(vgs_ctx* c) {
   if (!c->pt_labels_pending) return VGS_OK;
   c->pt_labels_pending = false;
   VGS_HIP_TRY(c, hipSetDevice(c->device));
   if (c->d2h_open && c->d2h_src == c->pt_label.p) { VGS_HIP_TRY(c, hipEventSynchronize(c->ev_d2h)); c->d2h_open = false; }
-  const int TB = 256;
-  hipLaunchKernelGGL(k_point_labels, dim3((unsigned)((c->N + TB - 1) / TB)), dim3(TB), 0, c->stream, c->perm_b.p, c->pt_vox.p, c->vox_label.p,
-                     c->N, c->pt_label.p);
+  { vgs_status sw = vgs_write_point_labels(c, false, c->pt_label.p); if (sw != VGS_OK) return sw; }
   VGS_HIP_TRY(c, hipEventRecord(c->ev[15], c->stream));
   c->labels_event_valid = true;
   VGS_HIP_TRY(c, hipStreamSynchronize(c->stream));
@@ -518,8 +624,7 @@
     const int cb_lut = c->cb_R;
     const uint32_t* cb_bits = use_bits ? c->conn_bits.p : (const uint32_t*)nullptr;
     const LcGate g_first = {(c->lc_tail.open && c->lc_tail.gated) ? (const unsigned int*)(c->counters.p + 57) : (const unsigned int*)nullptr, LC_FEW};
-    const size_t first_lds = (c->lc_tail.open && c->K.cross_lds_kb > 0) ? (size_t)c->K.cross_lds_kb * 1024 : 0;
-    hipLaunchKernelGGL(k_cross, dim3(vgs_xcd_grid((U + CX_ROWS - 1) / CX_ROWS)), dim3(64), first_lds, c->stream, c->used_ids.p, c->used_rank.p, U, c->adj_key.p, c->adj_cnt.p,
+    const size_t first_lds = (c->lc_tail.open && c->K.cross_lds_kb > 0) ? (size_t)c->K.cross_lds_kb * 1024 : 0;    hipLaunchKernelGGL(k_cross, dim3(vgs_xcd_grid((U + CX_ROWS - 1) / CX_ROWS)), dim3(64), first_lds, c->stream, c->used_ids.p, c->used_rank.p, U, c->adj_key.p, c->adj_cnt.p,
                        c->adj_stride, c->conn.p, mutual, c->csize.p, c->parent.p, gt, c->adj_gstride, c->adj_nrank.p, inv_res2,
                        c->lc_tail.open ? c->lc_pending.p : (const uint8_t*)nullptr, c->lc_defer.p, d_ndefer, (const uint32_t*)nullptr, 0,
                        cb_off, cb_lut, cb_bits, c->cb_words, early_union ? c->lc_defer_flag.p : (uint8_t*)nullptr, g_first, owned_early);
@@ -635,9 +740,10 @@
   hipLaunchKernelGGL(k_voxel_labels, dim3(nbV), dim3(TB), 0, c->stream, c->parent.p, keep_flag, c->kept_rank.p, V, c->vox_label.p,
                      (unsigned int*)(mcnt + 3));
   c->pt_labels_pending = c->have_region && N > 0;
-  if (!c->pt_labels_pending)
-    hipLaunchKernelGGL(k_point_labels, dim3((unsigned)((N + TB - 1) / TB)), dim3(TB), 0, c->stream, c->perm_b.p, c->pt_vox.p, c->vox_label.p,
-                       N, c->pt_label.p);
+  {
+    vgs_status sw = c->pt_labels_pending ? vgs_point_voxel_in_ready(c, false, nullptr) : vgs_write_point_labels(c, false, c->pt_label.p);
+    if (sw != VGS_OK) return sw;
+  }
   VGS_HIP_TRY(c, hipEventRecord(c->ev[15], c->stream));
   c->labels_event_valid = true;
   VGS_HIP_TRY(c, hipGetLastError());
diff --git a/vgs-svgs-segmentation_amd/csrc/multigpu.hip b/vgs-svgs-segmentation_amd/csrc/multigpu.hip
--- a/vgs-svgs-segmentation_amd/csrc/multigpu.hip
+++ b/vgs-svgs-segmentation_amd/csrc/multigpu.hip
@@ -103,14 +103,6 @@
   int64_t v = (int64_t)blockIdx.x * blockDim.x + threadIdx.x;
   if (v >= V) return;
   vox_label[v] = root_label[parent[v]];
-}
-
-__global__ void k_point_labels2(const uint32_t* __restrict__ perm, const uint32_t* __restrict__ pt_vox, const int32_t* __restrict__ vox_label,
-                                int64_t N, int32_t* __restrict__ label) {
-  int64_t j = (int64_t)blockIdx.x * blockDim.x + threadIdx.x;
-  if (j >= N) return;
-  const uint32_t v = pt_vox[j];
-  label[perm[j]] = (v == 0xffffffffu) ? -1 : vox_label[v];
 }
 
 __global__ void k_bnd_heads(const uint64_t* __restrict__ code_sorted, int64_t n, uint32_t* __restrict__ head) {
@@ -409,7 +401,7 @@
   if (c->stage < ST_SEGMENTED || c->bnd_unique < 0) { c->err = "vgs_apply_tile_labels: vgs_get_boundary_roots first"; return VGS_E_STATE; }
   VGS_HIP_TRY(c, hipSetDevice(c->device));
   if (c->d2h_open && c->d2h_src == c->pt_label.p) { VGS_HIP_TRY(c, hipEventSynchronize(c->ev_d2h)); c->d2h_open = false; }
-  const int64_t V = c->V, N = c->N;
+  const int64_t V = c->V;
   if (V == 0) return VGS_OK;
   const int TB = 256;
   VGS_HIP_TRY(c, c->root_label.ensure(V));
@@ -432,8 +424,7 @@
   }
   hipLaunchKernelGGL(k_apply_root_labels, dim3((unsigned)((V + TB - 1) / TB)), dim3(TB), 0, c->stream, c->parent.p, c->root_label.p, V,
                      c->vox_label.p);
-  hipLaunchKernelGGL(k_point_labels2, dim3((unsigned)((N + TB - 1) / TB)), dim3(TB), 0, c->stream, c->perm_b.p, c->pt_vox.p, c->vox_label.p, N,
-                     c->pt_label.p);
+  { vgs_status sw = vgs_write_point_labels(c, true, c->pt_label.p); if (sw != VGS_OK) return sw; }
   c->pt_labels_pending = false;
   VGS_HIP_TRY(c, hipEventRecord(c->ev[15], c->stream));
   c->labels_event_valid = true;
@@ -469,7 +460,7 @@
   if (c->stage < ST_SEGMENTED) { c->err = "vgs_apply_root_labels: segment first"; return VGS_E_STATE; }
   VGS_HIP_TRY(c, hipSetDevice(c->device));
   if (c->d2h_open && c->d2h_src == c->pt_label.p) { VGS_HIP_TRY(c, hipEventSynchronize(c->ev_d2h)); c->d2h_open = false; }
-  const int64_t V = c->V, N = c->N;
+  const int64_t V = c->V;
   if (V == 0) return VGS_OK;
   std::vector<int32_t> map((size_t)V, -1);
   for (int64_t k = 0; k < n_roots; ++k) {
@@ -481,8 +472,7 @@
   const int TB = 256;
   hipLaunchKernelGGL(k_apply_root_labels, dim3((unsigned)((V + TB - 1) / TB)), dim3(TB), 0, c->stream, c->parent.p, c->root_label.p, V,
                      c->vox_label.p);
-  hipLaunchKernelGGL(k_point_labels2, dim3((unsigned)((N + TB - 1) / TB)), dim3(TB), 0, c->stream, c->perm_b.p, c->pt_vox.p, c->vox_label.p, N,
-                     c->pt_label.p);
+  { vgs_status sw = vgs_write_point_labels(c, true, c->pt_label.p); if (sw != VGS_OK) return sw; }
   c->pt_labels_pending = false;
   VGS_HIP_TRY(c, hipEventRecord(c->ev[15], c->stream));
   c->labels_event_valid = true;
diff --git a/vgs-svgs-segmentation_amd/csrc/svgs.hip b/vgs-svgs-segmentation_amd/csrc/svgs.hip
--- a/vgs-svgs-segmentation_amd/csrc/svgs.hip
+++ b/vgs-svgs-segmentation_amd/csrc/svgs.hip
@@ -59,6 +59,7 @@
 vgs_status vgs_stage_svgs_group(vgs_ctx* c) {
   const int64_t N = c->N;
   c->V = 0; c->Nf = 0; c->U = 0;
+  { vgs_status sr = vgs_point_voxel_in_reset(c); if (sr != VGS_OK) return sr; }
   if (N == 0) { c->counts[VGS_N_FINITE] = 0; c->counts[VGS_N_VOXELS] = 0; c->counts[VGS_N_SUPERVOXELS] = 0; return VGS_OK; }
   VGS_HIP_TRY(c, c->sv_key_a.ensure(N)); VGS_HIP_TRY(c, c->sv_key_b.ensure(N));
   VGS_HIP_TRY(c, c->perm_a.ensure(N)); VGS_HIP_TRY(c, c->perm_b.ensure(N));
diff --git a/vgs-svgs-segmentation_amd/csrc/vgs_context.hpp b/vgs-svgs-segmentation_amd/csrc/vgs_context.hpp
--- a/vgs-svgs-segmentation_amd/csrc/vgs_context.hpp
+++ b/vgs-svgs-segmentation_amd/csrc/vgs_context.hpp
@@ -71,6 +71,7 @@
 };
 
 enum Stage { ST_NONE = 0, ST_POINTS = 1, ST_VOXELS = 2, ST_FEATURES = 3, ST_ADJACENCY = 4, ST_SEGMENTED = 5 };
+enum PviState { PVI_ABSENT = 0, PVI_QUEUED = 1, PVI_READY = 2 };
 
 struct VgsKnobs {
   int a1_max = 4;
@@ -99,6 +100,8 @@
   int pg_min_frac = 8;
   int pg_wide = 1;
   int pg_wide_frac = 8;
+  bool pvi_scatter = false;
+  int pvi_grid = 256;
   bool debug = false;
 };
 
@@ -142,6 +145,12 @@
   DevBuf<uint8_t> sort_tmp;
   DevBuf<uint64_t> grow_state;
   DevBuf<uint32_t> pt_vox;
+  DevBuf<uint32_t> pt_vox_in;
+  hipEvent_t ev_pvi = nullptr;
+  int pvi_state = PVI_ABSENT;
+  bool pvi_keys = false;
+  int pvi_key_bytes = 0, pvi_key_shift = 0;
+  bool bricks_current = false;
   DevBuf<uint32_t> vox_tile;
   DevBuf<uint32_t> head_flag;
   DevBuf<uint64_t> vox_code;
@@ -449,6 +458,10 @@
                                bool big_rows_too);
 vgs_status vgs_stage_localcut(vgs_ctx* c);
 vgs_status vgs_ensure_point_labels(vgs_ctx* c);
+vgs_status vgs_point_voxel_in_reset(vgs_ctx* c);
+vgs_status vgs_point_voxel_in_queue(vgs_ctx* c, hipStream_t s);
+vgs_status vgs_point_voxel_in_ready(vgs_ctx* c, bool make_absent, bool* ready);
+vgs_status vgs_write_point_labels(vgs_ctx* c, bool make_absent, int32_t* label);
 vgs_status vgs_localcut_finish_queue(vgs_ctx* c, hipStream_t s);
 vgs_status vgs_localcut_finish(vgs_ctx* c, hipStream_t s, unsigned int* n_deferred);
 vgs_status vgs_stage_merge(vgs_ctx* c);
diff --git a/vgs-svgs-segmentation_amd/csrc/voxelize.hip b/vgs-svgs-segmentation_amd/csrc/voxelize.hip
--- a/vgs-svgs-segmentation_amd/csrc/voxelize.hip
+++ b/vgs-svgs-segmentation_amd/csrc/voxelize.hip
@@ -468,13 +468,16 @@
   const uint64_t mask = (c->code_bits >= 64) ? ~0ull : ((1ull << c->code_bits) - 1ull);
   hipLaunchKernelGGL((k_voxel_runs<KeyT>), dim3((unsigned)n_tiles), dim3(VR_TB), 0, c->stream, code_b, N, pack_shift, tile_heads, mask, c->pt_vox.p,
                      c->vox_code.p, c->vox_start.p, v_total, (uint32_t)c->Nf);
+  c->pvi_keys = true; c->pvi_key_bytes = (int)sizeof(KeyT); c->pvi_key_shift = pack_shift;
   return VGS_OK;
 }
 
 vgs_status vgs_stage_voxelize(vgs_ctx* c) {
   const int64_t N = c->N;
   c->V = 0; c->Nf = 0; c->U = 0;
-  vgs_status st = grow_box(c);
+  vgs_status st = vgs_point_voxel_in_reset(c);
+  if (st != VGS_OK) return st;
+  st = grow_box(c);
   if (st != VGS_OK) return st;
   if (c->n_epochs == 0) {
     c->counts[VGS_N_FINITE] = 0; c->counts[VGS_N_VOXELS] = 0; c->counts[VGS_N_DEPTH] = 0;
@@ -486,6 +489,7 @@
   VGS_HIP_TRY(c, c->code_a.ensure(N)); VGS_HIP_TRY(c, c->code_b.ensure(N));
   VGS_HIP_TRY(c, c->perm_a.ensure(N)); VGS_HIP_TRY(c, c->perm_b.ensure(N));
   VGS_HIP_TRY(c, c->pt_vox.ensure(N));
+  if (c->P.method == 2) VGS_HIP_TRY(c, c->pt_vox_in.ensure(N));
   const int TB = 256;
   c->gathered = false;
   st = (c->code_bits + 1 <= 32) ? voxelize_sorted_table<uint32_t>(c) : voxelize_sorted_table<uint64_t>(c);
```

Result: no change. 1.699 billion (median of 6 runs) (+0.7%).
